# cokwa/bitHTM

Hardware: AMD Instinct MI355X
Metric: HTM timesteps/sec (SP + TM, learning on), 65536 cols x 32 cells (higher is better)
Workload: dtype u32 bit-packed / f64 + f32 permanences; 1 GPU; configs[2]: 65536 columns x 32 cells, SP + TM learning on, 1 MI355X; input_dim=1024, column_dim=65536, cell_dim=32, active_columns=1311, patterns=50, pretrain_steps=500, segments=96476, segment_slots=128, hip_graph=True, hip_graph_requested=True, pipelined=True, repetitions=15, streamed_calls=True

## Files before the change

bithtm_amd/_lib.py:

```python

import ctypes as C
import os

HERE = os.path.dirname(os.path.abspath(__file__))
LIB_PATH = os.path.join(HERE, "libbithtm_hip.so")
ABI_VERSION = 4


class HtmConfig(C.Structure):
    _fields_ = [
        ("struct_bytes", C.c_uint32), ("device", C.c_int32),
        ("input_dim", C.c_int32), ("column_dim", C.c_int32), ("cell_dim", C.c_int32),
        ("active_columns", C.c_int32), ("enable_sp", C.c_int32), ("enable_tm", C.c_int32),
        ("sp_permanence_threshold", C.c_double), ("sp_delta_on", C.c_double), ("sp_delta_off", C.c_double),
        ("boost_coefficient", C.c_float), ("duty_momentum", C.c_float), ("duty_increment", C.c_float),
        ("tm_learn_active", C.c_double), ("tm_learn_inactive", C.c_double),
        ("tm_punish_active", C.c_double), ("tm_punish_inactive", C.c_double),
        ("tm_learn_prune", C.c_int32), ("tm_punish_prune", C.c_int32),
        ("tm_permanence_initial", C.c_float), ("tm_permanence_threshold", C.c_float),
        ("segment_activation_threshold", C.c_int32), ("segment_matching_threshold", C.c_int32),
        ("segment_sampling_synapses", C.c_int32),
        ("segment_capacity", C.c_int32), ("segment_capacity_local", C.c_int32), ("segment_slots", C.c_int32),
        ("seed", C.c_uint32), ("shard_rank", C.c_int32), ("shard_world", C.c_int32), ("use_caller_stream", C.c_int32),
        ("stream", C.c_void_p),
    ]


class HtmInfo(C.Structure):
    _fields_ = [
        ("step_index", C.c_int64), ("segments", C.c_int32), ("local_segments", C.c_int32), ("matching_segments", C.c_int32),
        ("winner_cells", C.c_int32), ("active_cells", C.c_int32), ("has_distal_state", C.c_int32),
        ("has_winner_cells", C.c_int32), ("capacity_error", C.c_int32), ("words_per_row", C.c_int32),
        ("new_segment_requests", C.c_int32), ("recycled_segments", C.c_int32), ("appended_segments", C.c_int32),
        ("work_items", C.c_int32), ("select_fallbacks", C.c_int32), ("candidate_exact_steps", C.c_int32), ("hot_select_steps", C.c_int32),
        ("select_zoom_steps", C.c_int32),
    ]


class HtmStepRecord(C.Structure):
    _fields_ = [(name, C.c_int32) for name in (
        "active_columns", "bursting_columns", "predicted_columns_before", "predicted_columns", "active_cells", "winner_cells",
        "segments", "new_segments")]


class HtmRunRecord(C.Structure):
    _fields_ = [("struct_bytes", C.c_uint32), ("records", C.c_void_p), ("active_column", C.c_void_p), ("column_prediction", C.c_void_p)]


F_ACTIVE_COLUMN, F_OVERLAPS, F_BOOSTED, F_DUTY_CYCLE, F_CELL_ACTIVATION, F_CELL_PREDICTION = 1, 2, 3, 4, 5, 6
F_WINNER_WORDS, F_BURSTING, F_WINNER_CELL, F_SEG_CELL, F_SEG_NSYN, F_SEG_PRESYN, F_SEG_PERM = 7, 8, 9, 10, 11, 12, 13
F_SEGCOUNT, F_SEG_POTENTIAL, F_MATCH_SEGMENT, F_MATCH_INFO, F_MATCH_JITTER, F_CELL_MAX_JITTER = 14, 15, 16, 17, 18, 19
F_SEG_GID = 20
PLAN_GRAPH, PLAN_PIPELINED, PLAN_LEAN, PLAN_SCAN_LARGE = 1, 2, 4, 8
SP_OVERLAP, SP_BOOST, SP_SELECT, SP_ACTIVE, SP_LEARN, SP_DUTY, SP_COMMIT = 1, 2, 3, 4, 5, 6, 7

EXPORTS = {
    "htm_abi_version": (C.c_int, []),
    "htm_create": (C.c_int, [C.POINTER(HtmConfig), C.POINTER(C.c_void_p)]),
    "htm_destroy": (None, [C.c_void_p]),
    "htm_last_error": (C.c_char_p, [C.c_void_p]),
    "htm_sp_set_permanence": (C.c_int, [C.c_void_p, C.c_void_p, C.c_int32, C.c_int32]),
    "htm_set_epsilon": (C.c_int, [C.c_void_p, C.c_float]),
    "htm_sp_get_permanence": (C.c_int, [C.c_void_p, C.c_void_p, C.c_int32, C.c_int32]),
    "htm_step": (C.c_int, [C.c_void_p, C.c_void_p, C.c_int32]),
    "htm_sp_step": (C.c_int, [C.c_void_p, C.c_void_p, C.c_int32]),
    "htm_sp_phase": (C.c_int, [C.c_void_p, C.c_int32, C.c_void_p, C.c_int64]),
    "htm_tm_step": (C.c_int, [C.c_void_p, C.c_void_p, C.c_int32, C.c_int32, C.c_int32]),
    "htm_tm_update": (C.c_int, [C.c_void_p, C.c_void_p, C.c_void_p, C.c_void_p, C.c_int32, C.c_void_p]),
    "htm_tm_scan": (C.c_int, [C.c_void_p, C.c_void_p]),
    "htm_tm_run": (C.c_int, [C.c_void_p, C.c_void_p, C.c_int32, C.c_int32, C.c_int32, C.c_int32, C.c_int32, C.POINTER(HtmRunRecord)]),
    "htm_run": (C.c_int, [C.c_void_p, C.c_void_p, C.c_int32, C.c_int32, C.c_int32, C.c_int32]),
    "htm_prepare": (C.c_int, [C.c_void_p, C.c_void_p, C.c_int32, C.c_int32, C.c_int32, C.c_int32]),
    "htm_run_recorded": (C.c_int, [C.c_void_p, C.c_void_p, C.c_int32, C.c_int32, C.c_int32, C.c_int32, C.POINTER(HtmRunRecord)]),
    "htm_prepare_recorded": (C.c_int, [C.c_void_p, C.c_void_p, C.c_int32, C.c_int32, C.c_int32, C.c_int32]),
    "htm_reset": (C.c_int, [C.c_void_p]),
    "htm_set_run_resets": (C.c_int, [C.c_void_p, C.c_void_p, C.c_int32]),
    "htm_predicted_input": (C.c_int, [C.c_void_p, C.c_void_p]),
    "htm_set_run_predicted_input": (C.c_int, [C.c_void_p, C.c_void_p]),
    "htm_graph_count": (C.c_int, [C.c_void_p]),
    "htm_run_plan": (C.c_int, [C.c_void_p, C.c_int32, C.c_int32]),
    "htm_bank_upload": (C.c_int, [C.c_void_p, C.c_void_p, C.c_int32, C.POINTER(C.c_void_p)]),
    "htm_shard_record_bytes": (C.c_int64, [C.c_void_p]),
    "htm_shard_begin": (C.c_int, [C.c_void_p, C.c_void_p, C.c_int32, C.c_void_p, C.c_int32, C.c_void_p]),
    "htm_shard_finish": (C.c_int, [C.c_void_p, C.c_void_p, C.c_int32]),
    "htm_shard_unique_id": (C.c_int, [C.c_void_p]),
    "htm_shard_comm_init": (C.c_int, [C.c_void_p, C.c_void_p]),
    "htm_shard_step": (C.c_int, [C.c_void_p, C.c_void_p, C.c_int32, C.c_void_p, C.c_int32]),
    "htm_shard_comm_size": (C.c_int, [C.c_void_p]),
    "htm_shard_graph_ok": (C.c_int, [C.c_void_p]),
    "htm_shard_run": (C.c_int, [C.c_void_p, C.c_void_p, C.c_int32, C.c_int32, C.c_int32, C.c_int32]),
    "htm_shard_group_run": (C.c_int, [C.POINTER(C.c_void_p), C.c_int32, C.POINTER(C.c_void_p), C.c_int32, C.c_int32, C.c_int32, C.c_int32]),
    "htm_rccl_selftest": (C.c_int, [C.c_int32]),
    "htm_keyed_draws": (C.c_int, [C.c_uint32, C.c_int32, C.c_uint32, C.c_void_p, C.c_void_p, C.c_int64, C.c_void_p]),
    "htm_shard_group_step": (C.c_int, [C.POINTER(C.c_void_p), C.c_int32, C.POINTER(C.c_void_p), C.c_int32, C.c_void_p, C.c_int32]),
    "htm_populate": (C.c_int, [C.c_void_p, C.c_int64, C.c_int64, C.c_int32, C.c_int32, C.c_double, C.c_double, C.c_uint32]),
    "htm_sync": (C.c_int, [C.c_void_p]),
    "htm_get_stream": (C.c_int, [C.c_void_p, C.POINTER(C.c_void_p)]),
    "htm_get_info": (C.c_int, [C.c_void_p, C.POINTER(HtmInfo)]),
    "htm_read": (C.c_int64, [C.c_void_p, C.c_int32, C.c_void_p, C.c_int64]),
    "htm_read_rows": (C.c_int64, [C.c_void_p, C.c_int32, C.c_int64, C.c_int64, C.c_void_p, C.c_int64]),
    "htm_import_begin": (C.c_int, [C.c_void_p, C.c_int64]),
    "htm_write": (C.c_int, [C.c_void_p, C.c_int32, C.c_void_p, C.c_int64]),
    "htm_import_commit": (C.c_int, [C.c_void_p, C.c_int32, C.c_int32, C.c_int32, C.c_int32, C.c_int32]),
    "htm_profile": (C.c_int, [C.c_void_p, C.c_int32]),
    "htm_profile_read": (C.c_int, [C.c_void_p, C.c_int32, C.POINTER(C.c_char_p), C.POINTER(C.c_double),
                                   C.POINTER(C.c_int64)]),
    "htm_trace_read": (C.c_int64, [C.c_void_p, C.c_void_p, C.c_int64]),
    "htm_group_create": (C.c_int, [C.POINTER(C.c_void_p), C.c_int32, C.POINTER(C.c_void_p)]),
    "htm_group_destroy": (None, [C.c_void_p]),
    "htm_group_last_error": (C.c_char_p, [C.c_void_p]),
    "htm_group_run": (C.c_int, [C.c_void_p, C.POINTER(C.c_void_p), C.c_int32, C.c_int32, C.c_int32, C.c_int32, C.POINTER(HtmRunRecord)]),
    "htm_group_step": (C.c_int, [C.c_void_p, C.c_void_p, C.c_int32, C.POINTER(HtmRunRecord)]),
    "htm_create_view": (C.c_int, [C.c_void_p, C.POINTER(C.c_void_p)]),
    "htm_device_bytes": (C.c_int64, [C.c_void_p]),
    "htm_pack_columns": (C.c_int, [C.c_void_p, C.c_void_p, C.c_int32, C.c_int32, C.c_int32, C.c_void_p, C.c_int32, C.c_int32]),
    "htm_encode_votes": (C.c_int, [C.c_void_p, C.c_int32, C.c_int32, C.c_void_p, C.c_int32, C.c_int32]),
    "htm_set_run_feedback": (C.c_int, [C.c_void_p, C.c_void_p, C.c_int32, C.c_int32, C.c_int32]),
}

HIP_EXPORTS = {
    "hipSetDevice": (C.c_int, [C.c_int]),
    "hipMalloc": (C.c_int, [C.POINTER(C.c_void_p), C.c_size_t]),
    "hipFree": (C.c_int, [C.c_void_p]),
    "hipMemcpy": (C.c_int, [C.c_void_p, C.c_void_p, C.c_size_t, C.c_int]),
    "hipGetErrorString": (C.c_char_p, [C.c_int]),
    "hipStreamCreateWithFlags": (C.c_int, [C.POINTER(C.c_void_p), C.c_uint]),
    "hipStreamDestroy": (C.c_int, [C.c_void_p]),
}
HIP_MEMCPY_HOST_TO_DEVICE = 1
HIP_MEMCPY_DEVICE_TO_HOST = 2

_lib = None


def load():
# ... 21 lines not shown
```

bithtm_amd/csrc/htm_dev.h:

```cpp
#ifndef BITHTM_HTM_DEV_H
#define BITHTM_HTM_DEV_H

typedef unsigned long long u64;

#define SEL_MAX_PASSES 6
#define SEL_DIGIT 12
#define SEL_BINS 4096
#define HIST_REP 4
#define SEL_COARSE 64
#define COARSE_REP 16
#define COARSE_STRIDE 1024
#define FAN_COUNTERS 16
#define FAN_STRIDE 32
#define HIST0_FINE (HIST_REP * SEL_BINS)
#define HIST0_PAR (HIST0_FINE + COARSE_REP * COARSE_STRIDE)
#define RB 512
#define SCAN_SEGS 64
#define DEAD_CAP 256
#define SHARD_HOT_KEYS 4
#define CAND_CAP 256
#define WIN_LDS 4096
#define MAX_SLOTS 512
#define SYN_CONNECTED 0x80000000u
#define SYN_CELL 0x7FFFFFFF
#define SEG_BUSY 0x40000000
#define EPS32 1e-8f

#define KEY_SHIFT 3
__device__ __forceinline__ u64 select_key_bits(u64 bits) { return bits ? (bits - ((u64)(1023 - 150) << 52)) << KEY_SHIFT : 0ull; }
__device__ __forceinline__ u64 select_key(double boosted) { return select_key_bits((u64)__double_as_longlong(boosted)); }

#define WIN_COARSE 31
#define WIN_FINE 7
#define WIN_BINS (2 + (WIN_COARSE << WIN_FINE))
#define WIN_LOWBITS (52 - WIN_FINE)
static_assert(WIN_BINS <= SEL_BINS, "the window's bins fit the select histogram");
__host__ __device__ __forceinline__ uint32_t win_bin(u64 key, uint32_t base) {
    const uint32_t c = (uint32_t)(key >> 52);
    if (c < base) return 0u;
    const uint32_t o = c - base;
    return o >= WIN_COARSE ? 1u + (WIN_COARSE << WIN_FINE) : 1u + ((o << WIN_FINE) | ((uint32_t)(key >> WIN_LOWBITS) & ((1u << WIN_FINE) - 1u)));
}
__host__ __device__ __forceinline__ uint32_t win_base_for(u64 kth_key) {
    const uint32_t c = (uint32_t)(kth_key >> 52);
    return c > WIN_COARSE / 2 ? min(c - WIN_COARSE / 2, 4096u - WIN_COARSE) : 0u;
}

__host__ __device__ __forceinline__ uint32_t win_base_global(u64 kth_key) { return win_base_for(kth_key); }

__host__ __device__ __forceinline__ int sel_shift(int pass) { return pass < 5 ? 52 - SEL_DIGIT * pass : 0; }
__host__ __device__ __forceinline__ int sel_bits(int pass) { return pass < 5 ? SEL_DIGIT : 4; }

struct Counters {
    uint32_t step[2];
    int32_t S;
    int32_t n_win[2];
    int32_t has_winner[2];
    int32_t has_distal;
    uint32_t cm_dense_step;
    int32_t n_active_cells;
    alignas(128) int32_t n_work[2];
    int32_t n_bind[2];
    alignas(128) int32_t n_work_last;
    int32_t sel_fallbacks;
    int32_t cand_exact;
    int32_t hot_selects;
    int32_t sel_zooms;
    uint32_t emit_epoch;
    int32_t n_un;
    int32_t n_recycled, n_new, S_old;
    int32_t L;
    int32_t n_lfree;
    int32_t error;
    u64 sel_prefix[2];
    uint32_t sel_krem[2];
    uint32_t sel_win[2];
    uint32_t sel_win_global;
    u64 sel_pass_prefix[2][SEL_MAX_PASSES + 1];
    uint32_t sel_pass_krem[2][SEL_MAX_PASSES + 1];
};

struct Dev {
    int I, W, W4, Ipad, C, K, k, E, Scap, work_cap, sel_passes, colwords, low_zero, cand_d, cand_pairwise, cand_others, cand_speculate, cand_take_all, cand_zoom, poll_delay;
    int win_offset;
    int cls_rows_max;
    int LK, KP, WPC;
    int world, c0, c1;
    int sel_lo, sel_hi, sel_k;
    int Lcap, n_cand;
    int hot_budget, hot_target;
    int cand_cap;
    double sp_thr, sp_don, sp_doff;
    float coef, mom, dinc;
    double lrn_act, lrn_inact, pun_act, pun_inact;
    int lrn_prune, pun_prune;
    float perm_init, perm_thr;
    float eps;
    int act_thr, match_thr, sample;
    uint32_t seed;
    double *perm;
    uint32_t *mask;
    float *duty;
    int *overlap[2];
    double *boosted[2];
    u64 *key[2];
    uint32_t *hist;
    uint32_t *hist0;
    uint32_t *sel_blk;
    uint32_t *sel_rec;
    int *active_cols[2];
    uint32_t *input_stage;
    uint32_t *act[2];
    uint32_t *pred[2];
    uint32_t *win[2];
    uint32_t *colbits[2];
    int *winners[2];
    uint8_t *bursting;
    int *actw_id;
    uint32_t *winw_idx;
    uint8_t *actcnt;
    uint32_t *act_list;
    uint16_t *col_rank[2];
    uint32_t *unacc_word;
    uint32_t *fan;
    int *unacc_list;
    int *seg_cell;
    int *seg_nsyn;
    int *presyn;
    float *sperm;
    int *segcount;
    uint32_t *cellmax[2];
    uint32_t *match_bits[2];
    uint32_t *seg_info;
    float *seg_jit;
    uint32_t *work;
    int *recyc_cnt;
    int *recyc_cnt2;
    int *recyc_need;
    int *seg_gid;
    int *g2l;
    uint32_t *dead_bits;
    int *lfree;
    int *asg_gid;
    int *cand_cols;
    int *dead_list;
    const uint32_t *punish;
    unsigned char *send;
    Counters *ctr;
    unsigned long long *trace;
    uint32_t trace_until;
};

__device__ __forceinline__ int lane_id() { return threadIdx.x & 63; }
__device__ __forceinline__ u64 lanemask_lt() { return (1ull << lane_id()) - 1ull; }

__device__ __forceinline__ uint32_t wave_incl_scan(uint32_t v) {
    uint32_t t = v;
    t += (uint32_t)__builtin_amdgcn_update_dpp(0, (int)v, 0x111, 0xf, 0xf, false);
    t += (uint32_t)__builtin_amdgcn_update_dpp(0, (int)v, 0x112, 0xf, 0xf, false);
    t += (uint32_t)__builtin_amdgcn_update_dpp(0, (int)v, 0x113, 0xf, 0xf, false);
    t += (uint32_t)__builtin_amdgcn_update_dpp(0, (int)t, 0x114, 0xf, 0xe, false);
    t += (uint32_t)__builtin_amdgcn_update_dpp(0, (int)t, 0x118, 0xf, 0xc, false);
    t += (uint32_t)__builtin_amdgcn_update_dpp(0, (int)t, 0x142, 0xa, 0xf, false);
    t += (uint32_t)__builtin_amdgcn_update_dpp(0, (int)t, 0x143, 0xc, 0xf, false);
    return t;
}

__device__ __forceinline__ uint32_t wave_sum(uint32_t v) { return (uint32_t)__builtin_amdgcn_readlane((int)wave_incl_scan(v), 63); }

#ifdef BITHTM_BISECT_A
__device__ __forceinline__ uint32_t wave_read(uint32_t v, int src) { return (uint32_t)__shfl((int)v, src); }
__device__ __forceinline__ int wave_read(int v, int src) { return __shfl(v, src); }
#else
__device__ __forceinline__ uint32_t wave_read(uint32_t v, int src) { return (uint32_t)__builtin_amdgcn_readlane((int)v, src); }
__device__ __forceinline__ int wave_read(int v, int src) { return __builtin_amdgcn_readlane(v, src); }
#endif
__device__ __forceinline__ u64 wave_read(u64 v, int src) {
#ifdef BITHTM_BISECT_A
    return ((u64)(uint32_t)__shfl((int)(v >> 32), src) << 32) | (uint32_t)__shfl((int)(uint32_t)v, src);
#endif
    return ((u64)(uint32_t)__builtin_amdgcn_readlane((int)(v >> 32), src) << 32) | (uint32_t)__builtin_amdgcn_readlane((int)(uint32_t)v, src);
}

template <typename Op>
// ... 36 lines not shown
__device__ __forceinline__ void lds_barrier() { asm volatile("s_waitcnt lgkmcnt(0)\n\ts_barrier" ::: "memory"); }

template <typename Op>
__device__ __forceinline__ float half_reduce(float v, float ident, Op op) {
    const int id = __float_as_int(ident);
#define BITHTM_DPPF(src, ctrl, rm, bm) __int_as_float(__builtin_amdgcn_update_dpp(id, __float_as_int(src), ctrl, rm, bm, false))
    float t = v;
    t = op(t, BITHTM_DPPF(v, 0x111, 0xf, 0xf));
    t = op(t, BITHTM_DPPF(v, 0x112, 0xf, 0xf));
    t = op(t, BITHTM_DPPF(v, 0x113, 0xf, 0xf));
    t = op(t, BITHTM_DPPF(t, 0x114, 0xf, 0xe));
    t = op(t, BITHTM_DPPF(t, 0x118, 0xf, 0xc));
    t = op(t, BITHTM_DPPF(t, 0x142, 0xa, 0xf));
#undef BITHTM_DPPF
    const float lo = __int_as_float(__builtin_amdgcn_readlane(__float_as_int(t), 31));
    const float hi = __int_as_float(__builtin_amdgcn_readlane(__float_as_int(t), 63));
    return lane_id() < 32 ? lo : hi;
}

template <int BS, bool LDS_ONLY = false>
__device__ __forceinline__ uint32_t block_excl_scan(uint32_t v, uint32_t *s_wave, uint32_t &total) {
    const int lane = lane_id(), wv = threadIdx.x >> 6;
    const uint32_t x = wave_incl_scan(v);
    if (lane == 63) s_wave[wv] = x;
    if (LDS_ONLY) lds_barrier(); else __syncthreads();
    uint32_t woff = 0, tot = 0;
#pragma unroll
    for (int i = 0; i < BS / 64; ++i) {
        uint32_t t = s_wave[i];
        if (i < wv) woff += t;
        tot += t;
    }
    if (LDS_ONLY) lds_barrier(); else __syncthreads();
    total = tot;
    return woff + x - v;
}

__device__ __forceinline__ int wave_append(int *counter, bool pred) {
    u64 m = __ballot(pred);
    if (m == 0) return -1;
    int leader = __ffsll((long long)m) - 1;
    int base = 0;
    if (lane_id() == leader) base = atomicAdd(counter, __popcll(m));
    base = wave_read(base, leader);
    return pred ? base + __popcll(m & lanemask_lt()) : -1;
}

__device__ __forceinline__ void recyc_add(const Dev &d, int blk1024, int delta) {
    atomicAdd(&d.recyc_cnt[blk1024], delta);
    atomicAdd(&d.recyc_cnt2[blk1024 >> 10], delta);
}

__device__ __forceinline__ void hist_add(uint32_t *h, uint32_t digit, bool active) {
    u64 todo = __ballot(active);
    while (todo) {
        const int leader = __ffsll((long long)todo) - 1;
        const uint32_t dl = wave_read(digit, leader);
        const u64 same = __ballot(active && digit == dl) & todo;
        if (lane_id() == leader) atomicAdd(&h[dl], (uint32_t)__popcll(same));
        todo &= ~same;
    }
}

__device__ __forceinline__ void hist_add_tie(uint32_t *h, uint32_t digit, bool active) {
    const u64 act = __ballot(active);
    if (!act) return;
    const int leader = __ffsll((long long)act) - 1;
    const uint32_t dl = wave_read(digit, leader);
    const u64 same = __ballot(active && digit == dl);
    if (lane_id() == leader) atomicAdd(&h[dl], (uint32_t)__popcll(same));
    if (active && digit != dl) atomicAdd(&h[digit], 1u);
}

__device__ __forceinline__ u64 spread32(uint32_t v) {
    u64 x = v;
    x = (x | (x << 16)) & 0x0000FFFF0000FFFFull;
    x = (x | (x << 8)) & 0x00FF00FF00FF00FFull;
    x = (x | (x << 4)) & 0x0F0F0F0F0F0F0F0Full;
    x = (x | (x << 2)) & 0x3333333333333333ull;
    x = (x | (x << 1)) & 0x5555555555555555ull;
    return x;
}

__device__ __forceinline__ uint32_t cell_mask(int K) { return K >= 32 ? 0xFFFFFFFFu : ((1u << K) - 1u); }
__device__ __forceinline__ u64 cell_mask64(int K) { return K >= 64 ? ~0ull : ((1ull << K) - 1ull); }
__device__ __forceinline__ uint32_t cell_mask_word(int K, int h) { return cell_mask(K - 32 * h); }
__device__ __forceinline__ uint32_t enc_to_flat(const Dev &d, int enc) { return (uint32_t)((enc >> d.LK) * d.K + (enc & (d.KP - 1))); }

#endif
```

bithtm_amd/csrc/htm_engine.hip:

```cpp

#include <hip/hip_runtime.h>
#include <hip/hip_ext.h>
#include <dlfcn.h>
#include <stdint.h>
#include <stdio.h>
#include <string.h>
#include <algorithm>
#include <climits>
#include <chrono>
#include <map>
#include <mutex>
#include <string>
#include <tuple>
#include <type_traits>
#include <vector>

#include "../../include/bithtm_hip.h"
#include "htm_fexp.h"
#include "htm_rng.h"

#include "htm_dev.h"
#include "htm_sp_kernels.h"
#include "htm_tm_kernels.h"
#include "htm_pipeline.h"
#include "htm_record.h"
#include "htm_reset.h"
#include "htm_decode.h"
#include "htm_stack.h"
#include "htm_forecast.h"
#include "htm_group.h"
#include "htm_tm_feed.h"


struct ncclUniqueIdBytes { char internal[128]; };

static thread_local std::string g_create_error;
static int (*g_rccl_destroy)(void *) = nullptr;

struct Knobs {
    int graph_steps, eager_below;
    bool trace;
    uint32_t trace_until;
    int lean, lean2_classify, lean2_order, step_split, fuse_tm, shard_window, step_window, tail_rows, scan_large, scan_large_above, scan_dyn;
    int defer_tail, shared_scan, shared_members;
    int lean_overlap, lean_learn, lean_learn_large, lean_scan, lean_scan_large, scan_blocks, sel_launch_digits;
    int cand_d, cand_pairwise, cls_rows_max, win_offset, cand_zoom, cand_speculate, cand_take_all, poll_delay, cand_others;
};

struct Sizes {
    int G;
    int sp_blocks, sel_blocks, c256_blocks, s1024_blocks, scan_blocks, zero_blocks, cus;
    int lean_learn_blocks, lean_learn_blocks_large, lean_scan_blocks, lean_scan_blocks_large, lean_overlap_blocks, lean2_classify_blocks;
    int lean_resident_large;
    bool emit_fits, emit_fits_open;
    bool emit_fits_lean;
    int sel_passes_fused, sel_passes_full;
};

struct RunGraphKey {
    int p; bool recording, resetting, decoding, feeding; int learning; bool sp_done, next_sp, next_front, lean; int spec; bool large, emit_fused, wmode;
    int span; const void *bank; int n_inputs;
    auto tie() const { return std::tie(p, recording, resetting, decoding, feeding, learning, sp_done, next_sp, next_front, lean, spec, large, emit_fused, wmode, span, bank, n_inputs); }
    bool operator<(const RunGraphKey &o) const { return tie() < o.tie(); }
};

struct ShardGraphKey {
    int p, learning; bool front_done, front_next; int span, ranks, n_inputs; std::vector<std::tuple<int, bool, bool>> per_rank; const void *bank;
    auto tie() const { return std::tie(p, learning, front_done, front_next, span, ranks, n_inputs, per_rank, bank); }
    bool operator<(const ShardGraphKey &o) const { return tie() < o.tie(); }
};

struct TmRunGraphKey {
    int p; bool recording, resetting; int learning, spec; bool large; int span; const void *lists; int n_rows, n;
    auto tie() const { return std::tie(p, recording, resetting, learning, spec, large, span, lists, n_rows, n); }
    bool operator<(const TmRunGraphKey &o) const { return tie() < o.tie(); }
};

struct htm_handle {
    htm_config cfg;
    Dev d;
    Knobs knob;
    Sizes sz;
    int device;
    hipStream_t stream;
    bool own_stream;
    long long step_host;
    std::string err;
    std::vector<void *> allocs;
    int *d_cols_stage;
    int rank, world;
    const uint32_t *shard_bank;
    int shard_n_inputs = 1;
    bool shard_open;
    bool shard_graph_ok;
    int shard_front_wmode;
    std::map<ShardGraphKey, hipGraphExec_t> shard_graphs;
    void *rccl_comm;
    unsigned char *shard_send, *shard_recv;
    bool emit_fused, emit_fused_open;
    bool tail_pending;
    int tail_p;
    bool window_known;
    int seg_hint;
    int *seg_pinned;
    const uint32_t *ahead_bank;
    int ahead_n_inputs, ahead_learning;
    bool ahead_lean;
    int phase_active;
    bool import_keep;
    bool phase_open;
    RecDev *d_rec;
    bool recording;
    const uint32_t *reset_bits;
    int reset_n;
    ResetDev *d_reset;
    bool resetting;
    int32_t *pin_out;
    PinDev *d_pin;
    bool decoding;
    int32_t *d_pin_buf;
    uint32_t *feed_bank;
    int feed_n;
    FeedDev *d_feed;
    int32_t *d_feed_votes;
    bool feeding;
    std::map<RunGraphKey, hipGraphExec_t> graphs;
    std::map<TmRunGraphKey, hipGraphExec_t> tm_graphs;
    std::vector<int> imp_pot, imp_match_seg;
    std::vector<int> imp_seg_cell, imp_seg_nsyn, imp_presyn;
    std::vector<float> imp_perm;
    std::vector<uint32_t> imp_match_info;
    std::vector<float> imp_match_jit;
    bool profile;
    hipEvent_t prof_last;
    std::vector<hipEvent_t> prof_all;
// ... 217 lines not shown
        LAUNCH_ON(h, h->stream, lds, "tm_learn+tm_scan", kt_lse_plain[epl_slot(d)], n_learn + n_scan, 256, d, p, 0, n_learn, n_scan, spec);
    } else {
        launch_learn(h, p);
        launch_scan(h, p, scan_lds(d, 1) <= 64 * 1024);
    }
}

static void flush_tail(htm_handle *h) {
    if (!h->tail_pending) return;
    h->tail_pending = false;
    hipSetDevice(h->device);
    enqueue_tm_tail(h, h->tail_p);
}

static decltype(&k_learn_scan_tail<1>) const kt_learn_scan_tail[4] = {k_learn_scan_tail<1>, k_learn_scan_tail<2>, k_learn_scan_tail<4>, k_learn_scan_tail<8>};

static void enqueue_tm(htm_handle *h, int n_active, int learning, int want_winner, int p,
                       const uint32_t *bank, int n_inputs, bool sp_rows, int front_wmode = -1, bool defer_tail = false) {
    Dev &d = h->d;
    const int n_cls = learning ? kClassifyBlocks : 0;
    const bool fuse = tm_tail_fused(h);
    int n_sp_rows = (sp_rows && learning && h->cfg.enable_sp) ? d.k : 0;
    const int n_tail_rows = (fuse && h->world == 1 && h->knob.tail_rows && !defer_tail) ? n_sp_rows : 0;
    if (n_tail_rows) n_sp_rows = 0;
    const int n_duty = h->world > 1 ? (d.c1 - d.c0 + 255) / 256 : 0;
    LAUNCH(h, "tm_mid", k_mid_rows, 1 + n_cls + n_sp_rows + n_duty + h->sz.zero_blocks, 256, d, p, n_active, want_winner, learning, n_cls, bank, n_inputs, n_sp_rows, 0, n_duty);
    if (defer_tail) { h->tail_pending = true; h->tail_p = p; return; }
    if (fuse && (front_wmode >= 0 || n_tail_rows)) {
        const int epl = learn_epl(d), n_learn = h->sz.lean_learn_blocks, n_scan = h->sz.lean_scan_blocks, spec = scan_spec_blocks(h);
        const size_t lds = std::max(std::max(learn_lds(epl, 256), scan_lds(d, 1)), (size_t)SEL_BINS * 4);
        const int grid = n_learn + n_scan + (n_tail_rows ? n_tail_rows : h->sz.lean_overlap_blocks);
        const char *name = n_tail_rows ? "tm_learn+tm_scan+sp_learn" : "tm_learn+tm_scan+shard_overlap";
        LAUNCH_ON(h, h->stream, lds, name, kt_learn_scan_tail[epl_slot(d)], grid, 256, d, p, n_learn, n_scan, spec, bank, n_inputs, h->sz.G, front_wmode, n_tail_rows);
        return;
    }
    enqueue_tm_tail(h, p);
    if (front_wmode >= 0)
        LAUNCH(h, "shard_overlap", k_shard_overlap, h->sz.sp_blocks, RB, d, bank, n_inputs, h->sz.G, p, front_wmode, 1);
}

struct StepPlan { bool sp_done, next_sp, next_front; };

static bool can_pipeline(const htm_handle *h) {
    return h->cfg.enable_sp && h->cfg.enable_tm && h->world == 1 && h->emit_fused_open && h->d.sel_passes == 2;
}

static bool can_lean(const htm_handle *h) {
    return h->knob.lean && can_pipeline(h) && scan_lds(h->d, 1) <= 64 * 1024 && h->sz.emit_fits_lean;
}

static decltype(&k_learn_scan_emit<1, 6>) const kt_lse_large[4] = {k_learn_scan_emit<1, 4, false>, k_learn_scan_emit<2, 4, false>,
                                                                   k_learn_scan_emit<4, 4, false>, k_learn_scan_emit<8, 4, false>};
static decltype(&k_learn_scan_emit<1, 6>) const kt_lse_tab[4] = {k_learn_scan_emit<1, 6, true>, k_learn_scan_emit<2, 6, true>,
                                                                 k_learn_scan_emit<4, 6, true>, k_learn_scan_emit<8, 6, true>};
static decltype(&k_learn_scan_emit<1, 6>) lse_kernel(const Dev &d, int form) {
    return (form == LSE_TAB ? kt_lse_tab : form == LSE_LARGE ? kt_lse_large : kt_lse_plain)[epl_slot(d)];
}

static int lse_form(const htm_handle *h) { return scan_pool_is_large(h) ? LSE_LARGE : lean_tab(h->d) ? LSE_TAB : LSE_PLAIN; }

static void launch_learn_scan_emit(htm_handle *h, int p, int n_emit) {
    Dev &d = h->d;
    const int epl = learn_epl(d);
    const size_t lds = std::max(std::max(learn_lds(epl, 256), lean_scan_lds(d)), sizeof(EmitShared));
    const bool large = scan_pool_is_large(h), dyn = large && h->knob.scan_dyn > 0;
    const int n_learn = dyn ? h->sz.lean_learn_blocks_large : h->sz.lean_learn_blocks;
    int n_scan = large ? h->sz.lean_scan_blocks_large : h->sz.lean_scan_blocks;
    if (dyn) n_scan = std::max(64, h->sz.lean_resident_large - n_emit - n_learn);
    const int grid = n_emit + n_learn + n_scan;
    if (large && !dyn) n_scan = -n_scan;
    const int spec = dyn ? 0 : scan_spec_blocks(h);
    const char *lse_name = large ? "tm_learn+tm_scan_large+sp_emit" : "tm_learn+tm_scan+sp_emit";
    LAUNCH_ON(h, h->stream, lds, lse_name, lse_kernel(d, lse_form(h)), grid, 256, d, p, n_emit, n_learn, n_scan, spec);
}

static int lean2_classify_blocks(const htm_handle *h, int learning) {
    if (!learning) return 0;
    return scan_pool_is_large(h) && !h->knob.lean2_classify ? std::max(h->sz.lean2_classify_blocks, 192) : h->sz.lean2_classify_blocks;
}

static void enqueue_lean(htm_handle *h, int p, int learning, const uint32_t *bank, int n_inputs, StepPlan plan) {
    Dev &d = h->d;
    const int n_act = (d.k * d.KP + 255) / 256, n_rows = learning ? d.k : 0;
    const int n_cls = learning ? kClassifyBlocks : 0, n_ov = plan.next_sp ? h->sz.lean_overlap_blocks : 0;
    if (h->knob.lean == 2) {
        const int n_cls2 = lean2_classify_blocks(h, learning);
        const int n_duty = n_ov ? 0 : h->sz.c256_blocks, n_clear = d.WPC * h->sz.c256_blocks;
        LAUNCH_ON(h, h->stream, (size_t)SEL_BINS * 4, "tm_activate+tm_mid+sp_learn+sp_overlap", k_act_mid_rows,
                  n_act + 1 + n_cls2 + n_rows + n_ov + n_duty + n_clear + h->sz.zero_blocks, 256, d, p, d.k, n_act, learning, n_cls2, bank, n_inputs, n_rows, h->sz.G, n_ov,
                  n_duty, n_clear, h->knob.lean2_order);
    } else {
        LAUNCH(h, "tm_activate+sp_learn", k_act_rows, n_act + n_rows + (1 + d.WPC) * h->sz.c256_blocks, 256, d, p, d.k, n_act, bank, n_inputs, n_rows, h->sz.c256_blocks);
        LAUNCH_ON(h, h->stream, (size_t)SEL_BINS * 4, "tm_mid+sp_overlap", k_mid_overlap, 1 + n_cls + n_ov + h->sz.zero_blocks, 256, d, p, d.k, 1, learning, n_cls,
                  bank, n_inputs, h->sz.G, n_ov);
    }
    launch_learn_scan_emit(h, p, plan.next_sp ? h->sz.c256_blocks : 0);
}

static decltype(&k_learn_overlap<1>) const kt_learn_overlap[4] = {k_learn_overlap<1>, k_learn_overlap<2>, k_learn_overlap<4>, k_learn_overlap<8>};
static decltype(&k_scan_sel<true, 1>) const kt_scan_sel[4] = {k_scan_sel<true, 1>, k_scan_sel<false, 1>, k_scan_sel<true, 6>, k_scan_sel<false, 6>};

static void enqueue_pipelined(htm_handle *h, int p, int learning, const uint32_t *bank, int n_inputs, StepPlan plan) {
    Dev &d = h->d;
    const int n_cls = learning ? kClassifyBlocks : 0;
    const int n_emit = plan.next_sp ? h->sz.c256_blocks : 0;
    LAUNCH_ON(h, h->stream, sizeof(EmitShared), "tm_activate+sp_emit", k_open_emit, n_emit + (d.k * d.KP + 255) / 256, 256, d, p, n_emit, d.k);
    const int n_rows = (plan.next_sp && learning) ? d.k : 0, n_duty = plan.next_sp ? h->sz.c256_blocks : 0;
    LAUNCH(h, "tm_mid+sp_learn", k_mid_rows, 1 + n_cls + n_rows + n_duty + h->sz.zero_blocks, 256, d, p, d.k, 1, learning, n_cls, bank, n_inputs, n_rows, 1, n_duty);
    LAUNCH_ON(h, h->stream, std::max(learn_lds(learn_epl(d)), (size_t)SEL_BINS * 4), "tm_learn+sp_overlap", kt_learn_overlap[epl_slot(d)],
              kLearnBlocks + (plan.next_front ? h->sz.sp_blocks : 0), RB, d, p, kLearnBlocks, bank, n_inputs, h->sz.G, p, 2);
    const bool use_lds = scan_lds(d, 1) <= 64 * 1024, large = scan_pool_is_large(h);
    const int n_sel = plan.next_front ? 64 : 0, n_clear = plan.next_sp ? h->sz.c256_blocks : 0;
    LAUNCH_ON(h, h->stream, std::max(scan_lds(d, use_lds), sizeof(SelShared)), large ? "tm_scan_large+sp_select" : "tm_scan+sp_select",
              kt_scan_sel[scan_slot(large, use_lds)], h->sz.scan_blocks + n_sel + n_clear, 256, d, p, n_sel, n_clear, p, scan_spec_blocks(h));
}

static void enqueue_cold_start(htm_handle *h, const uint32_t *bank, int n_inputs, int learning, StepPlan plan) {
    Dev &d = h->d;
    const int p = (int)(h->step_host & 1);
    if (plan.sp_done || !plan.next_sp) return;
    const int wmode = step_wmode(h);
    if (can_lean(h)) {
        enqueue_sp_front(h, bank, n_inputs, p, wmode);
        enqueue_sp_back(h, bank, n_inputs, p, 1, 0, false, wmode);
        return;
    }
    enqueue_sp_front(h, bank, n_inputs, p, wmode);
    enqueue_sp_back(h, bank, n_inputs, p, 1, EMIT_DUTY | EMIT_CLEAR, learning != 0, wmode);
    LAUNCH(h, "sp_overlap", k_sp_overlap, h->sz.sp_blocks, RB, d, bank, n_inputs, h->sz.G, p, p ^ 1, 1, 0);
    LAUNCH(h, "sp_select", k_sel_pass, h->sz.sel_blocks, RB, d, 1, p ^ 1);
}

static int reset_blocks(const Dev &d) { return std::max(1, std::min(1024, (d.C * d.KP + 255) / 256)); }

static void enqueue_run_reset(htm_handle *h, int p) {
    if (h->resetting) LAUNCH(h, "tm_reset", k_tm_reset, reset_blocks(h->d), 256, h->d, p, h->d_reset, h->recording ? h->d_rec : nullptr, 0u);
}

static void enqueue_rest(htm_handle *h, int p, const uint32_t *bank, int n_inputs, int learning, StepPlan plan) {
    enqueue_run_reset(h, p);
    if ((plan.sp_done || plan.next_sp) && can_lean(h)) {
        enqueue_lean(h, p, learning, bank, n_inputs, plan);
    } else if (plan.sp_done || plan.next_sp) {
        enqueue_pipelined(h, p, learning, bank, n_inputs, plan);
    } else {
        enqueue_sp_back(h, bank, n_inputs, p, 1, EMIT_ALL, false, step_wmode(h));
        enqueue_tm(h, h->d.k, learning, 1, p, bank, n_inputs, true);
    }
}

static int rec_blocks(const Dev &d) { return std::max(REC_BLOCKS_MIN, (d.k + 255) / 256); }

static void enqueue_record(htm_handle *h, int p) {
    if (h->recording) LAUNCH(h, "record", k_rec_step, rec_blocks(h->d), 256, h->d, p, h->d_rec);
}

static void enqueue_decode(htm_handle *h, int p) {
    if (h->decoding) LAUNCH(h, "predicted_input", k_pin_step, pin_blocks(h->d.C), 256, h->d, p, (const PinDev *)h->d_pin);
}

static bool decode_unpipelined(const htm_handle *h) { return h->pin_out && !can_lean(h); }

static void enqueue_feed(htm_handle *h, int p) {
    if (!h->feeding) return;
    LAUNCH(h, "feedback_votes", k_feed_votes, pin_blocks(h->d.C), 256, h->d, p, (const FeedDev *)h->d_feed);
    LAUNCH(h, "feedback_encode", k_feed_step, 1, ENC_THREADS, h->d, p, (const FeedDev *)h->d_feed);
}

static int pin_begin_blocks(int n, int I) { return (int)std::max<size_t>(1, std::min<size_t>(1024, ((size_t)n * I + 255) / 256)); }

static int enqueue_step(htm_handle *h, const uint32_t *bank, int n_inputs, int learning, StepPlan plan, const uint32_t *host_input = nullptr) {
    if (!plan.sp_done && !plan.next_sp) enqueue_sp_front(h, bank, n_inputs, (int)(h->step_host & 1), step_wmode(h), host_input);
    enqueue_cold_start(h, bank, n_inputs, learning, plan);
    enqueue_rest(h, (int)(h->step_host & 1), bank, n_inputs, learning, plan);
    enqueue_record(h, (int)(h->step_host & 1));
    enqueue_decode(h, (int)(h->step_host & 1));
    enqueue_feed(h, (int)(h->step_host & 1));
    h->step_host += 1;
    return launch_status(h->err);
}

extern "C" int htm_abi_version(void) { return BITHTM_ABI_VERSION; }

extern "C" const char *htm_last_error(const htm_handle *h) { return h ? h->err.c_str() : g_create_error.c_str(); }

extern "C" void htm_destroy(htm_handle *h) {
    if (!h) return;
    {
        std::lock_guard<std::mutex> lock(g_registry_mutex);
        g_registry.erase(std::remove(g_registry.begin(), g_registry.end(), h), g_registry.end());
    }
    hipSetDevice(h->device);
    hipStreamSynchronize(h->stream);
    for (auto &kv : h->graphs) hipGraphExecDestroy(kv.second);
    for (auto &kv : h->shard_graphs) hipGraphExecDestroy(kv.second);
    for (auto &kv : h->tm_graphs) hipGraphExecDestroy(kv.second);
    for (auto &v : h->prof_events)
        for (auto &pr : v) { hipEventDestroy(pr.first); hipEventDestroy(pr.second); }
    for (hipEvent_t e : h->prof_all) hipEventDestroy(e);
    if (h->rccl_comm && g_rccl_destroy) g_rccl_destroy(h->rccl_comm);
    for (void *p : h->allocs) hipFree(p);
    for (void *p : h->weight_allocs) hipFree(p);
    if (h->seg_pinned) hipHostFree(h->seg_pinned);
    if (h->own_stream) hipStreamDestroy(h->stream);
    if (HtmShared *sh = h->shared) {
        bool last;
        {
            std::lock_guard<std::mutex> lock(g_shared_mutex);
            if (sh->parent == h) sh->parent = nullptr;
            last = --sh->refs == 0;
        }
        if (last) {
            for (void *p : sh->allocs) hipFree(p);
            if (sh->own_stream) hipStreamDestroy(sh->stream);
            delete sh;
        }
    }
    delete h;
}

static int fail_create(htm_handle *h, const std::string &msg, int code) {
    g_create_error = msg;
    if (h) { h->err = msg; htm_destroy(h); }
    return code;
}

static int alloc_weights(htm_handle *h) {
    Dev &d = h->d;
    const htm_config *cfg = &h->cfg;
    const size_t C = d.C;
    int rc = 0;
    if (cfg->enable_sp) {
        rc |= dalloc_weights(h, &d.perm, C * d.Ipad);
        rc |= dalloc_weights(h, &d.mask, C * d.W);
    }
    if (cfg->enable_tm) {
        const size_t S = d.Lcap, E = d.E, KP = d.KP;
        rc |= dalloc_weights(h, &d.seg_cell, S);
        rc |= dalloc_weights(h, &d.seg_nsyn, S);
        rc |= dalloc_weights(h, &d.presyn, S * E);
        rc |= dalloc_weights(h, &d.sperm, S * E);
        rc |= dalloc_weights(h, &d.segcount, C * KP);
    }
    return rc;
}

static int alloc_stream_state(htm_handle *h) {
    Dev &d = h->d;
    const htm_config *cfg = &h->cfg;
    const int world = h->world;
    int rc = 0;
    const size_t C = d.C, k = d.k;
    rc |= dalloc(h, &d.ctr, 1);
    rc |= dalloc(h, &d.active_cols[0], k + 8);
    rc |= dalloc(h, &d.active_cols[1], k + 8);
    if (cfg->enable_sp) {
        rc |= dalloc(h, &d.duty, C);
        for (int q = 0; q < 2; ++q) {
            rc |= dalloc(h, &d.overlap[q], C);
            rc |= dalloc(h, &d.boosted[q], C);
            rc |= dalloc(h, &d.key[q], C);
        }
        rc |= dalloc(h, &d.hist, (size_t)2 * SEL_MAX_PASSES * SEL_BINS);
        rc |= dalloc(h, &d.hist0, (size_t)2 * HIST0_PAR);
        rc |= dalloc(h, &d.sel_blk, (C + 255) / 256);
        rc |= dalloc(h, &d.sel_rec, (C + 255) / 256 * 32);
        rc |= dalloc(h, &d.input_stage, (size_t)d.W);
    }
    if (cfg->enable_tm) {
        const size_t S = d.Lcap, G = d.Scap;
        const size_t KP = d.KP, WPC = d.WPC;
        for (int q = 0; q < 2; ++q) {
            rc |= dalloc(h, &d.act[q], C * WPC);
            rc |= dalloc(h, &d.pred[q], C * WPC);
            rc |= dalloc(h, &d.winners[q], k * KP);
        }
        rc |= dalloc(h, &d.win[0], C * WPC);
        rc |= dalloc(h, &d.win[1], C * WPC);
        d.colwords = (int)((C + 63) / 64) * 2;
        const size_t colwords_padded = (size_t)((C + 255) / 256) * 8;
        rc |= dalloc(h, &d.colbits[0], colwords_padded);
        rc |= dalloc(h, &d.colbits[1], colwords_padded);
        rc |= dalloc(h, &d.bursting, k);
        rc |= dalloc(h, &d.actw_id, k * WPC + 8);
        rc |= dalloc(h, &d.winw_idx, k * WPC + 8);
        rc |= dalloc(h, &d.actcnt, k * WPC + 8);
        rc |= dalloc(h, &d.act_list, k * WPC + 16);
        rc |= dalloc(h, &d.col_rank[0], colwords_padded);
        rc |= dalloc(h, &d.col_rank[1], colwords_padded);
        rc |= dalloc(h, &d.unacc_word, k * WPC + 8);
        rc |= dalloc(h, &d.fan, (size_t)2 * FAN_COUNTERS * FAN_STRIDE);
        rc |= dalloc(h, &d.unacc_list, k * KP);
        for (int q = 0; q < 2; ++q) {
            rc |= dalloc(h, &d.cellmax[q], C * KP);
            rc |= dalloc(h, &d.match_bits[q], (S + 255) / 256 * 8);
        }
        rc |= dalloc(h, &d.seg_info, S);
        rc |= dalloc(h, &d.seg_jit, S);
        rc |= dalloc(h, &d.work, (size_t)d.work_cap);
        rc |= dalloc(h, &d.recyc_cnt, (G + 1023) / 1024);
        rc |= dalloc(h, &d.recyc_cnt2, ((G + 1023) / 1024 + 1023) / 1024 + 1);
        rc |= dalloc(h, &d.recyc_need, 2 * k * KP);
        rc |= dalloc(h, &d.dead_list, (size_t)1 + DEAD_CAP);
        if (world > 1) {
            rc |= dalloc(h, &d.seg_gid, S);
            rc |= dalloc(h, &d.g2l, G);
            rc |= dalloc(h, &d.dead_bits, (G + 31) / 32 + 32);
            rc |= dalloc(h, &d.lfree, S);
            rc |= dalloc(h, &d.asg_gid, k * 32);
            rc |= dalloc(h, &d.cand_cols, (size_t)d.n_cand + 8);
            if (!rc && (hipMemsetAsync(d.seg_gid, 0xFF, S * 4, h->stream) != hipSuccess ||
                        hipMemsetAsync(d.g2l, 0xFF, G * 4, h->stream) != hipSuccess)) { h->err = "hipMemsetAsync failed"; rc = HTM_ERR_HIP; }
        }
        rc |= dalloc(h, &h->d_cols_stage, k);
    }
    if (h->knob.trace) rc |= dalloc(h, &d.trace, (size_t)8 * 4096 * 2);
    return rc;
}

static const char *env_str(const char *name) { return getenv(name); }
static int env_int(const char *name, int dflt, int lo = INT_MIN, int hi = INT_MAX) {
    const char *e = env_str(name);
    return e ? std::max(lo, std::min(hi, atoi(e))) : dflt;
}
static int env_flag(const char *name, int dflt) {
    const char *e = env_str(name);
    return e ? atoi(e) != 0 : dflt;
}

static Knobs read_knobs() {
    Knobs k;
    k.graph_steps = env_int("BITHTM_GRAPH_STEPS", 16, 1, 256);
    k.eager_below = env_int("BITHTM_EAGER_BELOW", 64, 0);
    k.trace = env_str("BITHTM_TRACE") != nullptr;
    const char *until = env_str("BITHTM_TRACE_UNTIL");
    k.trace_until = until ? (uint32_t)strtoul(until, nullptr, 10) : 0xFFFFFFFFu;
    k.lean = env_int("BITHTM_LEAN", 2, 0, 2);
    k.lean2_classify = env_int("BITHTM_LEAN2_CLASSIFY", 0, 1);
    k.step_split = env_flag("BITHTM_STEP_SPLIT", 1);
    {
        const char *e = env_str("BITHTM_LEAN2_ORDER");
        const int o = e ? (int)strtol(e, nullptr, 16) : 0x0312;
        int seen = 0, pos[4] = {-1, -1, -1, -1};
        for (int i = 0; i < 4; ++i) { const int r = (o >> (4 * (3 - i))) & 15; if (r < 4) { seen |= 1 << r; pos[r] = i; } }
        k.lean2_order = (o >= 0 && o <= 0x3333 && seen == 15 && pos[0] < pos[1]) ? o : 0x0312;
    }
    k.fuse_tm = env_flag("BITHTM_FUSE_TM", 1);
    k.shard_window = env_flag("BITHTM_SHARD_WINDOW", 1);
    k.scan_large = env_int("BITHTM_SCAN_LARGE", -1);
    k.scan_large_above = env_int("BITHTM_SCAN_LARGE_ABOVE", 3 * 1536 * SCAN_SEGS, 0);
    k.step_window = env_flag("BITHTM_STEP_WINDOW", 1);
    k.tail_rows = env_flag("BITHTM_TAIL_ROWS", 1);
    k.scan_dyn = env_flag("BITHTM_SCAN_DYN", 1);
    k.defer_tail = env_flag("BITHTM_DEFER_TAIL", 1);
    k.shared_scan = env_flag("BITHTM_SHARED_SCAN", 0);
    k.shared_members = env_int("BITHTM_SHARED_SCAN_MEMBERS", 0, 0);
    k.lean_overlap = env_int("BITHTM_LEAN_OVERLAP", 0, 1);
    k.lean_learn = env_int("BITHTM_LEAN_LEARN", 0, 1);
    k.lean_learn_large = env_int("BITHTM_LEAN_LEARN_LARGE", 0, 1);
    k.lean_scan = env_int("BITHTM_LEAN_SCAN", 0, 1);
    k.lean_scan_large = env_int("BITHTM_LEAN_SCAN_LARGE", 0, 1);
    k.scan_blocks = env_int("BITHTM_SCAN_BLOCKS", 0, 1);
    k.sel_launch_digits = env_int("BITHTM_SEL_LAUNCH_DIGITS", -1, 0);
    k.cand_d = env_int("BITHTM_CAND_D", CAND_D, 0, CAND_D);
    k.cand_pairwise = env_int("BITHTM_CAND_PAIRWISE", CAND_PAIRWISE, 0);
    k.cls_rows_max = env_int("BITHTM_CLASSIFY_WORDS_ABOVE", -1, 0);
    k.win_offset = env_int("BITHTM_SEL_WINDOW_OFFSET", 0, 0);
    k.cand_zoom = env_int("BITHTM_CAND_ZOOM", -1);
    k.cand_speculate = env_flag("BITHTM_CAND_SPECULATE", 1);
    k.cand_take_all = env_flag("BITHTM_CAND_TAKE_ALL", 1);
    k.poll_delay = env_int("BITHTM_POLL_DELAY", 7, 0, 64);
    k.cand_others = env_int("BITHTM_CAND_OTHERS", CAND_OTHERS, 0, CAND_OTHERS);
    return k;
}

static void size_launches(htm_handle *h) {
    Dev &d = h->d;
    const Knobs &k = h->knob;
    Sizes &z = h->sz;
    z.G = 1;
    while (z.G < d.W4 && z.G < 64) z.G <<= 1;
    const int rows_per_block = (RB / 64) * 4 * (64 / z.G);
    z.sp_blocks = std::max(1, std::min((d.c1 - d.c0 + rows_per_block - 1) / rows_per_block, 256));
    z.sel_blocks = std::max(1, std::min((d.sel_hi - d.sel_lo + RB - 1) / RB, 128));
    z.c256_blocks = (d.sel_hi - d.sel_lo + 255) / 256;
    z.s1024_blocks = std::max(1, (d.Scap + 1023) / 1024);
    z.scan_blocks = std::max(1, std::min((d.Lcap + SCAN_SEGS - 1) / SCAN_SEGS, 2048));
    if (z.scan_blocks > 256) z.scan_blocks = (z.scan_blocks + 255) & ~255;
    z.zero_blocks = std::max(1, std::min((d.Lcap / 128 + 4095) / 4096, 1024));
    z.lean_overlap_blocks = k.lean_overlap ? k.lean_overlap : z.sp_blocks * (RB / 256);
    z.lean_learn_blocks = k.lean_learn ? k.lean_learn : 512;
    z.lean_learn_blocks_large = k.lean_learn_large ? k.lean_learn_large : k.lean_learn ? z.lean_learn_blocks : 768;
    z.lean_scan_blocks = k.lean_scan ? k.lean_scan : (z.scan_blocks > 512 ? std::max(256, (z.scan_blocks * 3 / 8 + 255) & ~255) : z.scan_blocks);
    z.lean_scan_blocks_large = k.lean_scan_large ? k.lean_scan_large : k.lean_scan ? z.lean_scan_blocks : z.scan_blocks;
    if (k.scan_blocks) z.scan_blocks = k.scan_blocks;
    hipDeviceProp_t prop;
    const bool have_prop = hipGetDeviceProperties(&prop, h->device) == hipSuccess;
    z.cus = have_prop ? prop.multiProcessorCount : 256;
    int B = 0;
    while ((1ll << B) <= (long long)d.I) ++B;
    const int informative = std::min(64, 64 - (29 - B) - KEY_SHIFT);
    d.sel_passes = std::max(1, std::min(SEL_MAX_PASSES, (informative + SEL_DIGIT - 1) / SEL_DIGIT));
    d.low_zero = 64 - informative;
    int per_cu_emit = 0, per_cu_open = 0;
    if (have_prop && hipOccupancyMaxActiveBlocksPerMultiprocessor(&per_cu_emit, (const void *)k_sp_emit, 256, 0) == hipSuccess &&
        hipOccupancyMaxActiveBlocksPerMultiprocessor(&per_cu_open, (const void *)k_open_emit, 256, sizeof(EmitShared)) == hipSuccess) {
        z.emit_fits = z.c256_blocks <= std::min(1024, per_cu_emit * z.cus);
        z.emit_fits_open = z.emit_fits && z.c256_blocks + (d.k * d.KP + 255) / 256 <= std::min(1024, per_cu_open * z.cus);
        int per_cu_lean = 1 << 30;
        z.lean_resident_large = 1 << 30;
        const size_t lean_lds = std::max(std::max(learn_lds(learn_epl(d), 256), lean_scan_lds(d)), sizeof(EmitShared));
        bool asked = h->cfg.enable_tm && z.emit_fits && lean_lds <= 64 * 1024;
        for (int form = LSE_TAB; asked && form <= LSE_LARGE; ++form) {
            if (form == LSE_TAB && !lean_tab(d)) continue;
            int per_cu = 0;
            asked = hipOccupancyMaxActiveBlocksPerMultiprocessor(&per_cu, (const void *)lse_kernel(d, form), 256, lean_lds) == hipSuccess;
            per_cu_lean = std::min(per_cu_lean, per_cu);
            if (asked && form == LSE_LARGE) z.lean_resident_large = per_cu * z.cus;
        }
        z.emit_fits_lean = asked && z.c256_blocks <= std::min(1024, per_cu_lean * z.cus);
        if (z.lean_resident_large == (1 << 30)) z.lean_resident_large = 4 * z.cus;
    } else {
        (void)hipGetLastError();
        z.emit_fits = z.emit_fits_open = z.emit_fits_lean = false;
        z.lean_resident_large = 1024;
    }
    if (k.lean2_classify) {
        z.lean2_classify_blocks = k.lean2_classify;
    } else {
        int per_cu = 0, resident = 1536;
        if (have_prop && hipOccupancyMaxActiveBlocksPerMultiprocessor(&per_cu, (const void *)k_act_mid_rows, 256, (size_t)SEL_BINS * 4) == hipSuccess)
            resident = per_cu * z.cus;
        else
            (void)hipGetLastError();
        const int others = (d.k * d.KP + 255) / 256 + z.lean_overlap_blocks + d.k + 1;
        const int room = (resident - others) & ~7;
        z.lean2_classify_blocks = room >= 128 ? std::min(kClassifyBlocks, room) : 32;
    }
    z.sel_passes_full = d.sel_passes;
    z.sel_passes_fused = std::min(d.sel_passes, 2);
    if (k.sel_launch_digits >= 0) z.sel_passes_fused = std::max(2, std::min(d.sel_passes, k.sel_launch_digits));
}

extern "C" int htm_create(const htm_config *cfg, htm_handle **out) {
    if (!cfg || !out) return fail_create(nullptr, "htm_create: null argument", HTM_ERR_ARGUMENT);
    if (cfg->struct_bytes != sizeof(htm_config)) return fail_create(nullptr, "htm_create: htm_config size mismatch (ABI)", HTM_ERR_ARGUMENT);
    if (cfg->column_dim < 1 || cfg->active_columns < 1 || cfg->active_columns > cfg->column_dim)
        return fail_create(nullptr, "htm_create: need 1 <= active_columns <= column_dim", HTM_ERR_ARGUMENT);
    if (cfg->enable_sp && cfg->input_dim < 1) return fail_create(nullptr, "htm_create: input_dim < 1", HTM_ERR_ARGUMENT);
    if (cfg->enable_tm) {
        if (cfg->cell_dim < 1 || cfg->cell_dim > 64) return fail_create(nullptr, "htm_create: cell_dim must be in 1..64", HTM_ERR_ARGUMENT);
        if (cfg->segment_slots < 64 || cfg->segment_slots > MAX_SLOTS || cfg->segment_slots % 64)
            return fail_create(nullptr, "htm_create: segment_slots must be a multiple of 64 in 64..512", HTM_ERR_ARGUMENT);
        if (cfg->segment_capacity < 1) return fail_create(nullptr, "htm_create: segment_capacity < 1", HTM_ERR_ARGUMENT);
        if (cfg->segment_sampling_synapses < 1 || cfg->segment_sampling_synapses > 64)
            return fail_create(nullptr, "htm_create: segment_sampling_synapses must be in 1..64", HTM_ERR_ARGUMENT);
        if (cfg->segment_activation_threshold < cfg->segment_matching_threshold)
            return fail_create(nullptr, "htm_create: activation threshold < matching threshold", HTM_ERR_ARGUMENT);
        if ((long long)cfg->column_dim * (cfg->cell_dim > 32 ? 64 : 32) > 0x7FFFFFFFLL) return fail_create(nullptr, "htm_create: column_dim too large", HTM_ERR_ARGUMENT);
    }
    if (!cfg->enable_sp && !cfg->enable_tm) return fail_create(nullptr, "htm_create: nothing enabled", HTM_ERR_ARGUMENT);
    const int world = cfg->shard_world > 1 ? cfg->shard_world : 1;
    if (world > 1) {
        if (!cfg->enable_sp || !cfg->enable_tm) return fail_create(nullptr, "htm_create: a sharded handle needs SP and TM", HTM_ERR_ARGUMENT);
        if (cfg->cell_dim > 32) return fail_create(nullptr, "htm_create: a sharded handle takes cell_dim up to 32 (the exchange record carries one 32-bit word per column)", HTM_ERR_ARGUMENT);
        if (world > 64) return fail_create(nullptr, "htm_create: at most 64 shards", HTM_ERR_ARGUMENT);
        if (cfg->shard_rank < 0 || cfg->shard_rank >= world) return fail_create(nullptr, "htm_create: shard_rank out of range", HTM_ERR_ARGUMENT);
        if (cfg->column_dim % (world * 64)) return fail_create(nullptr, "htm_create: column_dim must be a multiple of 64 * shard_world", HTM_ERR_ARGUMENT);
    }

    htm_handle *h = new htm_handle();
    h->cfg = *cfg;
    h->device = cfg->device;
    h->rank = world > 1 ? cfg->shard_rank : 0;
    h->world = world;
    h->knob = read_knobs();
    hipError_t e = hipSetDevice(cfg->device);
    if (e != hipSuccess) return fail_create(h, std::string("hipSetDevice: ") + hipGetErrorString(e), HTM_ERR_HIP);
    if (cfg->use_caller_stream) {
        h->stream = (hipStream_t)cfg->stream;
    } else {
        e = hipStreamCreateWithFlags(&h->stream, hipStreamNonBlocking);
        if (e != hipSuccess) return fail_create(h, std::string("hipStreamCreate: ") + hipGetErrorString(e), HTM_ERR_HIP);
        h->own_stream = true;
    }
    Dev &d = h->d;
    d.I = cfg->enable_sp ? cfg->input_dim : 0;
    d.W = ((d.I + 127) / 128) * 4;
    d.W4 = d.W / 4;
    d.Ipad = d.W * 32;
    d.C = cfg->column_dim;
    d.world = world;
    d.c0 = h->rank * (d.C / world);
    d.c1 = d.c0 + d.C / world;
    d.K = cfg->enable_tm ? cfg->cell_dim : 0;
    d.KP = d.K > 32 ? 64 : 32;
    d.LK = d.K > 32 ? 6 : 5;
    d.WPC = d.KP / 32;
    d.k = cfg->active_columns;
    d.E = cfg->enable_tm ? cfg->segment_slots : 64;
    d.Scap = cfg->enable_tm ? cfg->segment_capacity : 0;
    d.Lcap = d.Scap;
    if (world > 1) {
        const long long dflt = std::min<long long>(d.Scap, 2LL * d.Scap / world + 1024);
        d.Lcap = cfg->segment_capacity_local > 0 ? std::min(cfg->segment_capacity_local, cfg->segment_capacity) : (int)dflt;
    }
    d.work_cap = d.Lcap + d.k * d.KP;
    d.sel_lo = d.c0; d.sel_hi = d.c1;
    d.sel_k = d.n_cand = std::min(d.k, d.c1 - d.c0);
    d.cand_cap = shard_cand_cap(d.n_cand, d.c1 - d.c0);
    d.hot_budget = std::max(1, std::min(d.cand_cap, (SHARD_HOT_KEYS * 1024) / std::max(world, 1)));
    d.hot_target = std::max(1, std::min(d.sel_k, d.hot_budget / 2));
    d.sp_thr = cfg->sp_permanence_threshold; d.sp_don = cfg->sp_delta_on; d.sp_doff = cfg->sp_delta_off;
    d.coef = cfg->boost_coefficient; d.mom = cfg->duty_momentum; d.dinc = cfg->duty_increment;
    d.lrn_act = cfg->tm_learn_active; d.lrn_inact = cfg->tm_learn_inactive;
    d.pun_act = cfg->tm_punish_active; d.pun_inact = cfg->tm_punish_inactive;
    d.lrn_prune = cfg->tm_learn_prune; d.pun_prune = cfg->tm_punish_prune;
    d.perm_init = cfg->tm_permanence_initial; d.perm_thr = cfg->tm_permanence_threshold;
    d.eps = EPS32;
    d.act_thr = cfg->segment_activation_threshold; d.match_thr = cfg->segment_matching_threshold;
    d.sample = cfg->segment_sampling_synapses;
    d.seed = cfg->seed;
    const Knobs &k = h->knob;
    d.trace_until = k.trace_until; d.cand_d = k.cand_d; d.cand_pairwise = k.cand_pairwise; d.cls_rows_max = k.cls_rows_max; d.win_offset = k.win_offset;
    d.cand_zoom = k.cand_zoom; d.cand_speculate = k.cand_speculate; d.cand_take_all = k.cand_take_all; d.poll_delay = k.poll_delay; d.cand_others = k.cand_others;
    int rc = alloc_weights(h);
    rc |= alloc_stream_state(h);
    if (rc) return fail_create(h, h->err, HTM_ERR_HIP);
    if (hipHostMalloc((void **)&h->seg_pinned, sizeof(int), hipHostMallocDefault) == hipSuccess) *h->seg_pinned = 0; else h->seg_pinned = nullptr;
    size_launches(h);
    e = hipStreamSynchronize(h->stream);
    if (e != hipSuccess) return fail_create(h, std::string("hipStreamSynchronize: ") + hipGetErrorString(e), HTM_ERR_HIP);
    {
        std::lock_guard<std::mutex> lock(g_registry_mutex);
        g_registry.push_back(h);
    }
    refresh_exchange_mode(h);
    *out = h;
    return HTM_OK;
}


#define REFUSE_ON_VIEW(h, what)                                                                                   \
    do {                                                                                                          \
        if ((h)->is_view) {                                                                                       \
            (h)->err = std::string(what) + ": not available on an inference view (it shares its parent's weights and never learns)"; \
            return HTM_ERR_STATE;                                                                                 \
        }                                                                                                         \
    } while (0)

static void weights_touched(htm_handle *h) {
    if (h->shared && !h->is_view) {
        std::lock_guard<std::mutex> lock(g_shared_mutex);
        h->shared->wgen += 1;
    }
}

static int view_enter(htm_handle *h, int learning) {
    if (!h->is_view) return 0;
    if (learning) { h->err = "an inference view steps with learning = 0 only (it shares its parent's weights)"; return HTM_ERR_STATE; }
    htm_handle *par;
    long long wgen;
    {
        std::lock_guard<std::mutex> lock(g_shared_mutex);
        par = h->shared->parent;
        wgen = h->shared->wgen;
    }
    HIPCHK(h, hipSetDevice(h->device));
    if (par) {
        flush_tail(par);
        if (sp_is_ahead(par)) {
            h->err = "the view's parent is ahead (its htm_run ended with HTM_RUN_CONTINUE): finish the parent's run first";
            return HTM_ERR_STATE;
        }
// ... 73 lines not shown
              hipMemsetAsync(d.ctr->n_bind, 0, sizeof(d.ctr->n_bind), h->stream) == hipSuccess &&
              hipMemsetAsync(&d.ctr->error, 0, sizeof(int32_t), h->stream) == hipSuccess;
    if (ok) {
        hipLaunchKernelGGL(k_tm_reset, dim3(reset_blocks(d)), dim3(256), 0, h->stream, d, (int)(h->step_host & 1), (const ResetDev *)nullptr,
                           (RecDev *)nullptr, (uint32_t)h->step_host);
        ok = hipGetLastError() == hipSuccess;
    }
    if (hipHostMalloc((void **)&h->seg_pinned, sizeof(int), hipHostMallocDefault) == hipSuccess) *h->seg_pinned = parent->seg_hint; else h->seg_pinned = nullptr;
    if (!ok || hipStreamSynchronize(h->stream) != hipSuccess) return fail_create(h, "htm_create_view: copying the parent's stream state failed", HTM_ERR_HIP);
    {
        std::lock_guard<std::mutex> lock(g_registry_mutex);
        g_registry.push_back(h);
    }
    refresh_exchange_mode(h);
    *out = h;
    return HTM_OK;
}

extern "C" int64_t htm_device_bytes(htm_handle *h) {
    if (!h) return HTM_ERR_ARGUMENT;
    return h->own_bytes;
}

extern "C" int htm_set_epsilon(htm_handle *h, float epsilon) {
    if (!h) return HTM_ERR_ARGUMENT;
    if (h) flush_tail(h);
    if (!(epsilon > 0.f) || epsilon > 1.f) { h->err = "htm_set_epsilon: need 0 < epsilon <= 1"; return HTM_ERR_ARGUMENT; }
    REJECT_WHEN_AHEAD(h);
    if (epsilon == h->d.eps) return HTM_OK;
    HIPCHK(h, hipSetDevice(h->device));
    HIPCHK(h, hipStreamSynchronize(h->stream));
    for (auto &kv : h->graphs) hipGraphExecDestroy(kv.second);
    h->graphs.clear();
    h->d.eps = epsilon;
    return HTM_OK;
}

extern "C" int htm_get_stream(htm_handle *h, void **stream) {
    if (!h || !stream) return HTM_ERR_ARGUMENT;
    *stream = (void *)h->stream;
    return HTM_OK;
}

extern "C" int htm_sync(htm_handle *h) {
    if (!h) return HTM_ERR_ARGUMENT;
    if (h) flush_tail(h);
    HIPCHK(h, hipSetDevice(h->device));
    const auto t0 = std::chrono::steady_clock::now();
    for (;;) {
        const hipError_t e = hipStreamQuery(h->stream);
        if (e == hipSuccess) return HTM_OK;
        if (e != hipErrorNotReady) { h->err = std::string("hipStreamQuery: ") + hipGetErrorString(e); return HTM_ERR_HIP; }
        if (std::chrono::steady_clock::now() - t0 > std::chrono::milliseconds(2)) break;
    }
    HIPCHK(h, hipStreamSynchronize(h->stream));
    return HTM_OK;
}

static int check_rows(htm_handle *h, const void *rows, int row_begin, int row_count) {
    if (!h) return HTM_ERR_ARGUMENT;
    if (!h->cfg.enable_sp) { h->err = "handle has no Spatial Pooler"; return HTM_ERR_STATE; }
    if (!rows || row_begin < 0 || row_count < 0 || row_begin + (long long)row_count > h->d.C) {
        h->err = "permanence rows out of range";
        return HTM_ERR_ARGUMENT;
    }
    return 0;
}

extern "C" int htm_sp_set_permanence(htm_handle *h, const double *rows, int32_t row_begin, int32_t row_count) {
    if (h) REFUSE_ON_VIEW(h, "htm_sp_set_permanence");
    if (h) flush_tail(h);
    if (h) weights_touched(h);
    int rc = check_rows(h, rows, row_begin, row_count);
    if (rc) return rc;
    REJECT_WHEN_AHEAD(h);
    if (row_count == 0) return HTM_OK;
    Dev &d = h->d;
    HIPCHK(h, hipSetDevice(h->device));
    HIPCHK(h, hipMemcpy2DAsync(d.perm + (size_t)row_begin * d.Ipad, (size_t)d.Ipad * 8, rows, (size_t)d.I * 8,
                               (size_t)d.I * 8, (size_t)row_count, hipMemcpyHostToDevice, h->stream));
    const long long waves = (long long)row_count * (d.Ipad / 64);
    const int blocks = (int)std::min<long long>((waves + 3) / 4, 8192);
    hipLaunchKernelGGL(k_sp_build_mask, dim3(blocks), dim3(256), 0, h->stream, d, row_begin, row_count);
    HIPCHK(h, hipStreamSynchronize(h->stream));
    return HTM_OK;
}

extern "C" int htm_sp_get_permanence(htm_handle *h, double *rows, int32_t row_begin, int32_t row_count) {
    if (h) flush_tail(h);
    int rc = check_rows(h, rows, row_begin, row_count);
    if (rc) return rc;
    REJECT_WHEN_AHEAD(h);
    if (row_count == 0) return HTM_OK;
    Dev &d = h->d;
    HIPCHK(h, hipSetDevice(h->device));
    HIPCHK(h, hipMemcpy2DAsync(rows, (size_t)d.I * 8, d.perm + (size_t)row_begin * d.Ipad, (size_t)d.Ipad * 8,
                               (size_t)d.I * 8, (size_t)row_count, hipMemcpyDeviceToHost, h->stream));
    HIPCHK(h, hipStreamSynchronize(h->stream));
    return HTM_OK;
}

static int close_open_phases(htm_handle *h) {
    if (!h->phase_open) return 0;
    const int p = (int)(h->step_host & 1);
    if (h->cfg.enable_sp) HIPCHK(h, hipMemsetAsync(h->d.hist0 + (size_t)p * HIST0_PAR, 0, (size_t)HIST0_PAR * 4, h->stream));
    h->phase_open = false;
    h->phase_active = 0;
    return 0;
}

static int stage_input(htm_handle *h, const uint32_t *packed_input) {
    Dev &d = h->d;
    const int words = (d.I + 31) / 32;
    HIPCHK(h, hipMemcpyAsync(d.input_stage, packed_input, (size_t)words * 4, hipMemcpyHostToDevice, h->stream));
    return 0;
}

static decltype(&k_learn_scan_front<1>) const kt_learn_scan_front[4] = {k_learn_scan_front<1>, k_learn_scan_front<2>, k_learn_scan_front<4>, k_learn_scan_front<8>};

extern "C" int htm_step(htm_handle *h, const uint32_t *packed_input, int32_t learning) {
    if (!h || !packed_input) return HTM_ERR_ARGUMENT;
    REJECT_WHEN_AHEAD(h);
    if (!h->cfg.enable_sp || !h->cfg.enable_tm) { h->err = "htm_step needs a handle with SP and TM"; return HTM_ERR_STATE; }
    if (h->world > 1) { h->err = "sharded handle: use htm_shard_begin / htm_shard_finish"; return HTM_ERR_STATE; }
    HIPCHK(h, hipSetDevice(h->device));
    int rc = view_enter(h, learning);
    if (rc) return rc;
    if (learning) weights_touched(h);
    refresh_exchange_mode(h);
    rc = close_open_phases(h);
    if (rc) return rc;
    if (h->d.W > ARG_INPUT_WORDS) {
        flush_tail(h);
        rc = stage_input(h, packed_input);
        if (rc) return rc;
    }
    Dev &d = h->d;
    if (h->knob.defer_tail && d.W <= ARG_INPUT_WORDS && tm_tail_fused(h) && !h->profile) {
        const int p = (int)(h->step_host & 1), wmode = step_wmode(h);
        const bool ride_emit = h->knob.step_split && h->tail_pending && wmode && h->emit_fused && can_lean(h);
        bool emitted = false;
        if (ride_emit) {
            enqueue_sp_front(h, d.input_stage, 1, p, wmode, packed_input);
            h->tail_pending = false;
            launch_learn_scan_emit(h, h->tail_p, h->sz.c256_blocks);
            h->window_known = true;
            emitted = true;
        } else if (h->tail_pending) {
            PackedInputArg in;
            memset(&in, 0, sizeof(in));
            memcpy(in.w, packed_input, (size_t)((d.I + 31) / 32) * 4);
            const int epl = learn_epl(d), n_learn = h->sz.lean_learn_blocks, n_scan = h->sz.lean_scan_blocks, spec = scan_spec_blocks(h);
            const size_t lds = std::max(std::max(learn_lds(epl, 256), scan_lds(d, 1)), (size_t)(SEL_BINS + ARG_INPUT_WORDS) * 4);
            const int grid = n_learn + n_scan + h->sz.lean_overlap_blocks;
            h->tail_pending = false;
            LAUNCH_ON(h, h->stream, lds, "tm_learn+tm_scan+sp_overlap", kt_learn_scan_front[epl_slot(d)], grid, 256, d, h->tail_p, n_learn, n_scan, spec, in, h->sz.G, p, wmode);
            if (!wmode)
                for (int pass = 1; pass < d.sel_passes; ++pass) LAUNCH(h, "sp_select", k_sel_pass, h->sz.sel_blocks, RB, d, pass, p);
        } else {
            enqueue_sp_front(h, d.input_stage, 1, p, wmode, packed_input);
        }
        if (h->knob.step_split) {
            if (!emitted) enqueue_sp_back(h, d.input_stage, 1, p, 1, 0, false, wmode);
            const int lrn = learning ? 1 : 0;
            const int n_act = (d.k * d.KP + 255) / 256, n_rows = lrn ? d.k : 0;
            const int n_cls2 = lean2_classify_blocks(h, lrn);
            const int n_duty = h->sz.c256_blocks, n_clear = d.WPC * h->sz.c256_blocks;
            LAUNCH_ON(h, h->stream, 0, "tm_activate+tm_mid+sp_learn", k_act_mid_rows, n_act + 1 + n_cls2 + n_rows + n_duty + n_clear + h->sz.zero_blocks, 256,
                      d, p, d.k, n_act, lrn, n_cls2, d.input_stage, 1, n_rows, h->sz.G, 0, n_duty, n_clear, h->knob.lean2_order);
            h->tail_pending = true;
            h->tail_p = p;
        } else {
            enqueue_sp_back(h, d.input_stage, 1, p, 1, EMIT_ALL, false, wmode);
            enqueue_tm(h, d.k, learning ? 1 : 0, 1, p, d.input_stage, 1, true, -1, true);
        }
        h->step_host += 1;
        return launch_status(h->err);
    }
    flush_tail(h);
    return enqueue_step(h, h->d.input_stage, 1, learning ? 1 : 0, StepPlan{false, false, false}, packed_input);
}

extern "C" int htm_sp_step(htm_handle *h, const uint32_t *packed_input, int32_t learning) {
    if (!h || !packed_input) return HTM_ERR_ARGUMENT;
    if (h) flush_tail(h);
    REJECT_WHEN_AHEAD(h);
    if (!h->cfg.enable_sp) { h->err = "handle has no Spatial Pooler"; return HTM_ERR_STATE; }
    if (h->cfg.enable_tm) { h->err = "htm_sp_step: the handle also has a Temporal Memory; use htm_step"; return HTM_ERR_STATE; }
    HIPCHK(h, hipSetDevice(h->device));
    refresh_exchange_mode(h);
    int rc = close_open_phases(h);
    if (rc) return rc;
    rc = stage_input(h, packed_input);
    if (rc) return rc;
    const int p = (int)(h->step_host & 1);
    enqueue_sp_front(h, h->d.input_stage, 1, p, step_wmode(h));
    enqueue_sp_back(h, h->d.input_stage, 1, p, 0, EMIT_ALL, learning && !h->cfg.enable_tm, step_wmode(h));
    h->step_host += 1;
    return HTM_OK;
}

extern "C" int htm_sp_phase(htm_handle *h, int32_t phase, const void *data, int64_t count) {
    if (!h) return HTM_ERR_ARGUMENT;
    if (h) flush_tail(h);
    REJECT_WHEN_AHEAD(h);
    if (!h->cfg.enable_sp) { h->err = "handle has no Spatial Pooler"; return HTM_ERR_STATE; }
    if (h->world > 1) { h->err = "htm_sp_phase: not available on a column-sharded handle"; return HTM_ERR_STATE; }
    REFUSE_ON_VIEW(h, "htm_sp_phase");
    if (phase == HTM_SP_LEARN) weights_touched(h);
    HIPCHK(h, hipSetDevice(h->device));
    refresh_exchange_mode(h);
    Dev &d = h->d;
    const int p = (int)(h->step_host & 1);
    const int c256 = (d.C + 255) / 256;
    if (phase == HTM_SP_OVERLAP || phase == HTM_SP_BOOST || (phase == HTM_SP_SELECT && data))
        HIPCHK(h, hipMemsetAsync(d.hist0 + (size_t)p * HIST0_PAR, 0, (size_t)HIST0_PAR * 4, h->stream));
    switch (phase) {
        case HTM_SP_OVERLAP: {
            if (!data) return HTM_ERR_ARGUMENT;
            int rc = stage_input(h, (const uint32_t *)data);
            if (rc) return rc;
            LAUNCH(h, "sp_overlap", k_sp_overlap, h->sz.sp_blocks, RB, d, d.input_stage, 1, h->sz.G, p, p, 0, 0);
            break;
        }
        case HTM_SP_BOOST: {
            if (!data || count != d.C) { h->err = "htm_sp_phase(BOOST): need column_dim overlaps"; return HTM_ERR_ARGUMENT; }
            HIPCHK(h, hipMemcpyAsync(d.overlap[p], data, (size_t)d.C * 4, hipMemcpyHostToDevice, h->stream));
            HIPCHK(h, hipStreamSynchronize(h->stream));
            LAUNCH(h, "sp_keys", k_sp_keys, std::min((d.C + RB - 1) / RB, 256), RB, d, p, 1);
            break;
        }
        case HTM_SP_SELECT: {
            if (data) {
                if (count != d.C) { h->err = "htm_sp_phase(SELECT): need column_dim boosted overlaps"; return HTM_ERR_ARGUMENT; }
                HIPCHK(h, hipMemcpyAsync(d.boosted[p], data, (size_t)d.C * 8, hipMemcpyHostToDevice, h->stream));
                HIPCHK(h, hipStreamSynchronize(h->stream));
                LAUNCH(h, "sp_keys", k_sp_keys, std::min((d.C + RB - 1) / RB, 256), RB, d, p, 0);
            }
            for (int pass = 1; pass < d.sel_passes; ++pass) LAUNCH(h, "sp_select", k_sel_pass, h->sz.sel_blocks, RB, d, pass, p);
            enqueue_sp_back(h, d.input_stage, 1, p, 0, 0, false);
            break;
        }
        case HTM_SP_ACTIVE: {
            if ((!data && count) || count < 0 || count > d.k) { h->err = "htm_sp_phase(ACTIVE): at most active_columns columns"; return HTM_ERR_ARGUMENT; }
            std::vector<int> cols((const int *)data, (const int *)data + count);
            std::sort(cols.begin(), cols.end());
            for (int64_t i = 0; i < count; ++i)
                if (cols[i] < 0 || cols[i] >= d.C || (i && cols[i] == cols[i - 1])) { h->err = "htm_sp_phase(ACTIVE): bad column list"; return HTM_ERR_ARGUMENT; }
            if (count) HIPCHK(h, hipMemcpyAsync(d.active_cols[p], cols.data(), (size_t)count * 4, hipMemcpyHostToDevice, h->stream));
            HIPCHK(h, hipStreamSynchronize(h->stream));
            h->phase_active = (int)count;
            h->phase_open = true;
// ... 843 lines not shown
    HIPCHK(h, hipStreamSynchronize(h->stream));
    h->seg_hint = (int)(h->world > 1 ? own : total);
    if (h->seg_pinned) *h->seg_pinned = h->seg_hint;
    return HTM_OK;
}

extern "C" int htm_bank_upload(htm_handle *h, const uint32_t *host_inputs, int32_t n_inputs, uint32_t **device_bank) {
    if (!h || !host_inputs || n_inputs < 1 || !device_bank) return HTM_ERR_ARGUMENT;
    if (!h->cfg.enable_sp) { h->err = "handle has no Spatial Pooler"; return HTM_ERR_STATE; }
    Dev &d = h->d;
    HIPCHK(h, hipSetDevice(h->device));
    uint32_t *bank = nullptr;
    int rc = dalloc(h, &bank, (size_t)n_inputs * d.W);
    if (rc) return rc;
    const size_t words = (size_t)(d.I + 31) / 32;
    HIPCHK(h, hipMemcpy2DAsync(bank, (size_t)d.W * 4, host_inputs, words * 4, words * 4, (size_t)n_inputs,
                               hipMemcpyHostToDevice, h->stream));
    HIPCHK(h, hipStreamSynchronize(h->stream));
    *device_bank = bank;
    return HTM_OK;
}

static int read_counters(htm_handle *h, Counters *out) {
    HIPCHK(h, hipSetDevice(h->device));
    HIPCHK(h, hipStreamSynchronize(h->stream));
    HIPCHK(h, hipMemcpy(out, h->d.ctr, sizeof(Counters), hipMemcpyDeviceToHost));
    h->seg_hint = h->world > 1 ? out->L : out->S;
    if (h->seg_pinned) *h->seg_pinned = h->seg_hint;
    return 0;
}

extern "C" int htm_get_info(htm_handle *h, htm_info *out) {
    if (!h || !out) return HTM_ERR_ARGUMENT;
    if (h) flush_tail(h);
    Counters c;
    int rc = read_counters(h, &c);
    if (rc) return rc;
    const int q = (int)((h->step_host + 1) & 1);
    const int rows = h->world > 1 ? c.L : c.S;
    out->step_index = h->step_host;
    out->segments = c.S;
    out->local_segments = rows;
    out->matching_segments = 0;
    if (c.has_distal && rows > 0) {
        std::vector<uint32_t> bits(((size_t)rows + 31) / 32);
        HIPCHK(h, hipMemcpy(bits.data(), h->d.match_bits[q], bits.size() * 4, hipMemcpyDeviceToHost));
        for (int i = 0; i < rows; ++i) out->matching_segments += (bits[(size_t)i >> 5] >> (i & 31)) & 1u;
    }
    out->winner_cells = c.n_win[q];
    out->active_cells = c.n_active_cells;
    out->has_distal_state = c.has_distal;
    out->has_winner_cells = h->step_host > 0 ? c.has_winner[q] : 0;
    out->capacity_error = c.error;
    out->words_per_row = h->d.W;
    out->new_segment_requests = c.n_un;
    out->recycled_segments = c.n_un ? c.n_recycled : 0;
    out->appended_segments = c.n_un ? c.n_new : 0;
    out->work_items = c.n_work_last;
    out->select_fallbacks = c.sel_fallbacks;
    out->candidate_exact_steps = c.cand_exact;
    out->hot_select_steps = c.hot_selects;
    out->select_zoom_steps = c.sel_zooms;
    if (c.error) {
        h->err = std::string("capacity exhausted:") + ((c.error & 1) ? " segment pool (segment_capacity)" : "") +
                 ((c.error & 2) ? " synapse slots (segment_slots)" : "") + ((c.error & 4) ? " work list / growth staging" : "") +
                 ((c.error & 8) ? " dead-segment report (DEAD_CAP)" : "") +
                 ((c.error & 16) ? " (internal) block hand-off timed out in k_sp_emit" : "") +
                 ((c.error & 32) ? " (internal) the middle role's wait for the activation blocks timed out in k_act_mid_rows" : "") +
                 ((c.error & 64) ? " (not a capacity) htm_pack_columns met a column id outside this handle's input range" : "") +
                 ((c.error & 128) ? " (not a capacity) htm_tm_run met a list row with a repeated column id or one outside [0, column_dim): the results of its steps are invalid" : "");
        return HTM_ERR_CAPACITY;
    }
    return HTM_OK;
}

static inline int enc_flat(int enc, int K) { return K > 32 ? (enc >> 6) * K + (enc & 63) : (enc >> 5) * K + (enc & 31); }
static inline int flat_enc(int flat, int K) { return (flat / K) * (K > 32 ? 64 : 32) + (flat % K); }

extern "C" int64_t htm_read(htm_handle *h, int32_t field, void *dst, int64_t count) {
    if (!h || !dst) return HTM_ERR_ARGUMENT;
    if (h) flush_tail(h);
    const bool fixed_size = field == HTM_F_ACTIVE_COLUMN || field == HTM_F_OVERLAPS || field == HTM_F_BOOSTED || field == HTM_F_DUTY_CYCLE ||
                            field == HTM_F_CELL_ACTIVATION || field == HTM_F_CELL_PREDICTION || field == HTM_F_WINNER_WORDS ||
                            field == HTM_F_BURSTING || field == HTM_F_SEGCOUNT || field == HTM_F_CELL_MAX_JITTER;
    Counters c;
    memset(&c, 0, sizeof(c));
    int rc = 0;
    if (fixed_size) {
        HIPCHK(h, hipSetDevice(h->device));
        HIPCHK(h, hipStreamSynchronize(h->stream));
    } else {
        rc = read_counters(h, &c);
        if (rc) return rc;
    }
    Dev &d = h->d;
    const int q = (int)((h->step_host + 1) & 1);
    const int qs = h->phase_open ? (int)(h->step_host & 1) : q;
    const bool sp = h->cfg.enable_sp, tm = h->cfg.enable_tm;
    const int64_t C = d.C, K = d.K, S = h->world > 1 ? c.L : c.S, E = d.E, CW = (int64_t)d.C * d.WPC, KP = d.KP;
    auto need = [&](bool ok, int64_t n) -> int64_t {
        if (!ok) { h->err = "htm_read: field not available on this handle"; return HTM_ERR_STATE; }
        if (count < n) { h->err = "htm_read: buffer too small"; return HTM_ERR_ARGUMENT; }
        return n;
    };
    auto copy = [&](const void *src, int64_t n, size_t elem) -> int64_t {
        if (n > 0 && hipMemcpy(dst, src, (size_t)n * elem, hipMemcpyDeviceToHost) != hipSuccess) { h->err = "htm_read: hipMemcpy failed"; return HTM_ERR_HIP; }
        return n;
    };
    int64_t n;
    switch (field) {
        case HTM_F_ACTIVE_COLUMN: if ((n = need(true, d.k)) < 0) return n; return copy(d.active_cols[qs], n, 4);
        case HTM_F_OVERLAPS: REJECT_WHEN_AHEAD(h); if ((n = need(sp, C)) < 0) return n; return copy(d.overlap[qs], n, 4);
        case HTM_F_BOOSTED: REJECT_WHEN_AHEAD(h); if ((n = need(sp, C)) < 0) return n; return copy(d.boosted[qs], n, 8);
        case HTM_F_DUTY_CYCLE: REJECT_WHEN_AHEAD(h); if ((n = need(sp, C)) < 0) return n; return copy(d.duty, n, 4);
        case HTM_F_CELL_ACTIVATION: if ((n = need(tm, CW)) < 0) return n; return copy(d.act[q], n, 4);
        case HTM_F_CELL_PREDICTION: if ((n = need(tm, CW)) < 0) return n; return copy(d.pred[q], n, 4);
        case HTM_F_WINNER_WORDS: if ((n = need(tm, CW)) < 0) return n; return copy(d.win[q], n, 4);
        case HTM_F_BURSTING: if ((n = need(tm, d.k)) < 0) return n; return copy(d.bursting, n, 1);
        case HTM_F_SEG_NSYN: if ((n = need(tm, S)) < 0) return n; return copy(d.seg_nsyn, n, 4);
        case HTM_F_SEG_POTENTIAL:
        case HTM_F_MATCH_SEGMENT:
        case HTM_F_MATCH_INFO:
        case HTM_F_MATCH_JITTER: {
            if (!tm) { h->err = "htm_read: field not available on this handle"; return HTM_ERR_STATE; }
            if (field == HTM_F_SEG_POTENTIAL) {
                if ((n = need(true, S)) < 0) return n;
                if (S == 0) return 0;
                if (!c.has_distal) { memset(dst, 0, (size_t)S * 4); return S; }
                int *tmp = nullptr;
                if (hipMalloc((void **)&tmp, (size_t)S * 4) != hipSuccess) { h->err = "htm_read: hipMalloc failed"; return HTM_ERR_HIP; }
                hipLaunchKernelGGL(k_tm_potentials, dim3((unsigned)std::min<int64_t>((S * 8 + 255) / 256, 8192)), dim3(256), 0, h->stream, d, q, tmp, 0, (int)S);
                const bool ok = hipStreamSynchronize(h->stream) == hipSuccess && hipMemcpy(dst, tmp, (size_t)S * 4, hipMemcpyDeviceToHost) == hipSuccess;
                hipFree(tmp);
                if (!ok) { h->err = "htm_read: potentials kernel failed"; return HTM_ERR_HIP; }
                return S;
            }
            std::vector<uint32_t> bits(((size_t)S + 31) / 32, 0u);
            std::vector<uint32_t> info((size_t)S);
            std::vector<float> jit((size_t)S);
            if (S && c.has_distal && (hipMemcpy(bits.data(), d.match_bits[q], bits.size() * 4, hipMemcpyDeviceToHost) != hipSuccess ||
                                      hipMemcpy(info.data(), d.seg_info, (size_t)S * 4, hipMemcpyDeviceToHost) != hipSuccess ||
                                      hipMemcpy(jit.data(), d.seg_jit, (size_t)S * 4, hipMemcpyDeviceToHost) != hipSuccess)) { h->err = "htm_read: hipMemcpy failed"; return HTM_ERR_HIP; }
            auto is_matching = [&](int64_t i) { return (bits[(size_t)i >> 5] >> (i & 31)) & 1u; };
            int64_t m = 0;
            for (int64_t i = 0; i < S; ++i) m += is_matching(i);
            if ((n = need(true, m)) < 0) return n;
            m = 0;
            for (int64_t i = 0; i < S; ++i) {
                if (!is_matching(i)) continue;
                const uint32_t v = info[(size_t)i];
                if (field == HTM_F_MATCH_SEGMENT) ((int *)dst)[m] = (int)i;
                else if (field == HTM_F_MATCH_INFO) ((uint32_t *)dst)[m] = v & ~0x40000000u;
                else ((float *)dst)[m] = jit[(size_t)i];
                ++m;
            }
            return m;
        }
        case HTM_F_WINNER_CELL:
        case HTM_F_SEG_CELL: {
            const bool w = field == HTM_F_WINNER_CELL;
            if ((n = need(tm, w ? c.n_win[q] : S)) < 0) return n;
            if ((rc = (int)copy(w ? d.winners[q] : d.seg_cell, n, 4)) < 0) return rc;
            int *v = (int *)dst;
            for (int64_t i = 0; i < n; ++i) v[i] = enc_flat(v[i], (int)K);
            return n;
        }
        case HTM_F_SEG_PRESYN:
        case HTM_F_SEG_PERM: {
            if ((n = need(tm, S * E)) < 0) return n;
            std::vector<int> nsyn((size_t)S);
            if (S && hipMemcpy(nsyn.data(), d.seg_nsyn, (size_t)S * 4, hipMemcpyDeviceToHost) != hipSuccess) { h->err = "htm_read: hipMemcpy failed"; return HTM_ERR_HIP; }
            if ((rc = (int)copy(field == HTM_F_SEG_PRESYN ? (const void *)d.presyn : (const void *)d.sperm, n, 4)) < 0) return rc;
            for (int64_t s = 0; s < S; ++s)
                for (int64_t e = 0; e < E; ++e) {
                    const bool valid = e < nsyn[(size_t)s];
                    if (field == HTM_F_SEG_PRESYN) { int *v = (int *)dst + s * E + e; *v = valid ? enc_flat(*v & SYN_CELL, (int)K) : -1; }
                    else if (!valid) ((float *)dst)[s * E + e] = -1.0f;
                }
            return n;
        }
        case HTM_F_SEGCOUNT:
        case HTM_F_CELL_MAX_JITTER: {
            if ((n = need(tm, C * K)) < 0) return n;
            std::vector<uint32_t> tmp((size_t)C * KP);
            const void *src = field == HTM_F_SEGCOUNT ? (const void *)d.segcount : (const void *)d.cellmax[q];
            if (hipMemcpy(tmp.data(), src, tmp.size() * 4, hipMemcpyDeviceToHost) != hipSuccess) { h->err = "htm_read: hipMemcpy failed"; return HTM_ERR_HIP; }
            uint32_t *v = (uint32_t *)dst;
            for (int64_t col = 0; col < C; ++col)
                for (int64_t j = 0; j < K; ++j) v[col * K + j] = tmp[(size_t)col * KP + j];
            return n;
        }
        case HTM_F_SEG_GID: {
            if ((n = need(tm, S)) < 0) return n;
            if (d.seg_gid) return copy(d.seg_gid, n, 4);
            for (int64_t i = 0; i < n; ++i) ((int *)dst)[i] = (int)i;
            return n;
        }
// ... 879 lines not shown
```

bithtm_amd/csrc/htm_pipeline.h:

```cpp
#ifndef BITHTM_HTM_PIPELINE_H
#define BITHTM_HTM_PIPELINE_H

struct TraceScope {
    unsigned long long *t;
    __device__ TraceScope(const Dev &d, int slot) {
#if defined(BITHTM_LEARN_STAMPS) || defined(BITHTM_SCAN_STAMPS) || defined(BITHTM_EMIT_STAMPS) || defined(BITHTM_SHARD_STAMPS)
        t = nullptr;
        return;
#endif
        t = (d.trace && blockIdx.x < 4096 && d.ctr->step[slot >> 2] < d.trace_until) ? d.trace + ((size_t)slot * 4096 + blockIdx.x) * 2 : nullptr;
        if (t && threadIdx.x == 0) t[0] = wall_clock64();
    }
    __device__ ~TraceScope() { if (t && threadIdx.x == 0) t[1] = wall_clock64(); }
};

__global__ __launch_bounds__(256) void k_open_emit(Dev d, int p, int n_emit_blocks, int n_active) {
    TraceScope ts(d, 0 + 4 * p);
    if ((int)blockIdx.x < n_emit_blocks) {
        role_emit(d, p ^ 1, 1, 1, 0, blockIdx.x, n_emit_blocks, (EmitShared *)dyn_lds);
    } else {
        const int idx = ((int)blockIdx.x - n_emit_blocks) * tm_groups_per_block(d) + tm_group_of(d, threadIdx.x);
        const bool ok = idx < n_active;
        const int a = ok ? d.active_cols[p][idx] : 0;
        tm_activate_column(d, p, 1, ok, a, idx, tm_pred_words(d, p, ok, a));
// ... 72 lines not shown
    int b = blockIdx.x;
    if (b < n_act_blocks) {
        const int idx = b * tm_groups_per_block(d) + tm_group_of(d, threadIdx.x);
        const bool ok = idx < n_active;
        const int a = ok ? d.active_cols[p][idx] : 0;
        tm_activate_column(d, p, 1, ok, a, idx, tm_pred_words(d, p, ok, a));
        return;
    }
    b -= n_act_blocks;
    if (b < n_rows) {
        role_sp_row<256>(d, p, bank, n_inputs, 0, b, threadIdx.x);
        return;
    }
    b -= n_rows;
    const int c = b * 256 + (int)threadIdx.x;
    if (b < n_duty_blocks) {
        if (c < d.C) {
            float dc = d.duty[c] * d.mom;
            if ((d.colbits[p][c >> 5] >> (c & 31)) & 1u) dc = dc + d.dinc;
            d.duty[c] = dc;
        }
        return;
    }
    const int n_clear = (int)gridDim.x - n_act_blocks - n_rows - n_duty_blocks;
    for (int w = (b - n_duty_blocks) * 256 + (int)threadIdx.x; w < d.C * d.WPC; w += n_clear * 256) {
        const int cc = w >> (d.LK - 5);
        d.pred[p][w] = 0;
        if (!((d.colbits[p][cc >> 5] >> (cc & 31)) & 1u)) { d.act[p][w] = 0; d.win[p][w] = 0; }
    }
}

__global__ __launch_bounds__(256) void k_mid_overlap(Dev d, int p, int n_active, int want_winner, int learning, int n_cls,
                                                     const uint32_t *__restrict__ bank, int n_inputs, int G, int n_overlap_blocks) {
    TraceScope ts(d, 1 + 4 * p);
    int b = blockIdx.x;
    if (b <= n_cls) {
        role_mid<256>(d, p, n_active, want_winner, learning, b, n_cls);
        return;
    }
    b -= 1 + n_cls;
    if (b < n_overlap_blocks) {
        role_overlap<256>(d, bank, n_inputs, G, p, p ^ 1, 1, b, n_overlap_blocks, (uint32_t *)dyn_lds, 1);
        return;
    }
    b -= n_overlap_blocks;
    const int nz = (int)gridDim.x - 1 - n_cls - n_overlap_blocks;
    const int words4 = ((d.world > 1 ? d.ctr->L : d.ctr->S) + 127) >> 7;
    uint4 *mb = (uint4 *)d.match_bits[p];
    for (int i = b * 256 + (int)threadIdx.x; i < words4; i += nz * 256) mb[i] = make_uint4(0u, 0u, 0u, 0u);
}

__device__ __forceinline__ void fan_signal(const Dev &d, int p, int b) {
    asm volatile("s_waitcnt vmcnt(0)" ::: "memory");
    __syncthreads();
    if (threadIdx.x == 0)
        __hip_atomic_fetch_add(d.fan + (size_t)(p * FAN_COUNTERS + (b & (FAN_COUNTERS - 1))) * FAN_STRIDE, 1u, __ATOMIC_RELAXED, __HIP_MEMORY_SCOPE_AGENT);
}

__device__ __forceinline__ void fan_wait(const Dev &d, int p, uint32_t target) {
    if (threadIdx.x < 64) {
        for (int looks = 0;; ++looks) {
            uint32_t v = threadIdx.x < FAN_COUNTERS
                             ? __hip_atomic_load(d.fan + (size_t)(p * FAN_COUNTERS + (int)threadIdx.x) * FAN_STRIDE, __ATOMIC_RELAXED, __HIP_MEMORY_SCOPE_AGENT) : 0u;
            v = wave_sum(v);
            if (v >= target) break;
            if (looks >= (1 << 18)) {
                if (threadIdx.x == 0) atomicOr(&d.ctr->error, 32);
                break;
            }
#ifndef BITHTM_FAN_SLEEP
#define BITHTM_FAN_SLEEP 4
#endif
            __builtin_amdgcn_s_sleep(BITHTM_FAN_SLEEP);
        }
    }
    __syncthreads();
}

#ifndef BITHTM_LEAN2_WAVES
#define BITHTM_LEAN2_WAVES 8
#endif
__global__ __launch_bounds__(256, BITHTM_LEAN2_WAVES) void k_act_mid_rows(Dev d, int p, int n_active, int n_act_blocks, int learning, int n_cls,
                                                      const uint32_t *__restrict__ bank, int n_inputs, int n_rows, int G, int n_overlap_blocks,
                                                      int n_duty_blocks, int n_clear_blocks, int order) {
    TraceScope ts(d, 0 + 4 * p);
    int b = blockIdx.x;
    int role = 4;
#pragma unroll
    for (int i = 3; i >= 0 && role == 4; --i) {
        const int r = (order >> (4 * i)) & 15;
        const int n = r == 0 ? n_act_blocks : r == 1 ? 1 + n_cls : r == 2 ? n_rows : n_overlap_blocks;
        if (b < n) role = r; else b -= n;
    }
    if (role == 0) {
        const int idx = b * tm_groups_per_block(d) + tm_group_of(d, threadIdx.x);
        const bool ok = idx < n_active;
        const int a = ok ? d.active_cols[p][idx] : 0;
        tm_activate_column<true>(d, p, 1, ok, a, idx, tm_pred_words(d, p, ok, a));
        fan_signal(d, p, b);
        return;
    }
    if (role == 1) {
        role_mid<256>(d, p, n_active, 1, learning, b, n_cls, 1, [&]() { fan_wait(d, p, (uint32_t)n_act_blocks); });
        return;
    }
    if (role == 2) {
        if (n_overlap_blocks > 0) role_sp_row<256, true>(d, p, bank, n_inputs, 0, b, threadIdx.x);
        else role_sp_row<256>(d, p, bank, n_inputs, 0, b, threadIdx.x);
        return;
    }
    if (role == 3) {
        role_overlap<256>(d, bank, n_inputs, G, p, p ^ 1, 1, b, n_overlap_blocks, (uint32_t *)dyn_lds, 1, n_rows > 0 ? 2 : 1);
        return;
    }
    if (b < n_duty_blocks) {
        const int c = b * 256 + (int)threadIdx.x;
        if (c < d.C) {
            float dc = d.duty[c] * d.mom;
            if ((d.colbits[p][c >> 5] >> (c & 31)) & 1u) dc = dc + d.dinc;
            d.duty[c] = dc;
        }
        return;
    }
    b -= n_duty_blocks;
    if (b < n_clear_blocks) {
        for (int w = b * 256 + (int)threadIdx.x; w < d.C * d.WPC; w += n_clear_blocks * 256) {
            const int cc = w >> (d.LK - 5);
            d.pred[p][w] = 0;
            if (!((d.colbits[p][cc >> 5] >> (cc & 31)) & 1u)) { d.act[p][w] = 0; d.win[p][w] = 0; }
        }
        return;
    }
    b -= n_clear_blocks;
    const int nz = (int)gridDim.x - n_act_blocks - 1 - n_cls - n_rows - n_overlap_blocks - n_duty_blocks - n_clear_blocks;
    const int words4 = (d.ctr->S + 127) >> 7;
    uint4 *mb = (uint4 *)d.match_bits[p];
    for (int i = b * 256 + (int)threadIdx.x; i < words4; i += nz * 256) mb[i] = make_uint4(0u, 0u, 0u, 0u);
}

template <int EPL, int MINW, bool TAB = false>
__global__ __launch_bounds__(256, MINW) void k_learn_scan_emit(Dev d, int p, int n_emit_blocks, int n_learn_blocks, int n_scan_blocks, int n_spec) {
    TraceScope ts(d, 2 + 4 * p);
    constexpr bool LARGE = MINW < 6;
    static_assert(!(LARGE && TAB), "the streaming scan reads the cell words from memory");
    const bool dyn = LARGE && n_scan_blocks > 0;
    if (n_scan_blocks < 0) n_scan_blocks = -n_scan_blocks;
    if (blockIdx.x == gridDim.x - 1 && threadIdx.x < FAN_COUNTERS) d.fan[(size_t)(p * FAN_COUNTERS + (int)threadIdx.x) * FAN_STRIDE] = 0u;
    int b = blockIdx.x, scan_blk;
    if (b < n_emit_blocks) {
        role_emit(d, p ^ 1, 1, 1, 0, b, n_emit_blocks, (EmitShared *)dyn_lds, 1);
        if (!dyn) return;
        scan_blk = -1 - b;
    } else if (b < n_emit_blocks + n_learn_blocks) {
        role_learn<EPL, 256, true>(d, p, b - n_emit_blocks, n_learn_blocks, (LearnShared<EPL, 256> *)dyn_lds);
        if (!dyn) return;
        scan_blk = -1 - b;
    } else {
        scan_blk = b - n_emit_blocks - n_learn_blocks;
    }
    if (LARGE) role_scan<256, true, true, false, true>(d, p, scan_blk, n_scan_blocks, dyn ? n_emit_blocks + n_learn_blocks : 0, (uint32_t *)dyn_lds);
    else role_scan<256, true, false, TAB>(d, p, scan_blk, n_scan_blocks, n_spec, (uint32_t *)dyn_lds);
}

template <int EPL>
__global__ __launch_bounds__(256, 6) void k_learn_scan_tail(Dev d, int p, int n_learn_blocks, int n_scan_blocks, int n_spec,
                                                            const uint32_t *__restrict__ bank, int n_inputs, int G, int wmode, int n_rows) {
    int b = blockIdx.x;
    if (blockIdx.x == gridDim.x - 1 && threadIdx.x < FAN_COUNTERS) d.fan[(size_t)(p * FAN_COUNTERS + (int)threadIdx.x) * FAN_STRIDE] = 0u;
    if (b < n_learn_blocks) {
        role_learn<EPL, 256, true>(d, p, b, n_learn_blocks, (LearnShared<EPL, 256> *)dyn_lds);
        return;
    }
    b -= n_learn_blocks;
    if (b < n_scan_blocks) {
        role_scan<256, true, false, false>(d, p, b, n_scan_blocks, n_spec, (uint32_t *)dyn_lds);
        return;
    }
    b -= n_scan_blocks;
    if (n_rows > 0) role_sp_row<256>(d, p, bank, n_inputs, 0, b, threadIdx.x);
    else role_overlap<256>(d, bank, n_inputs, G, p, p ^ 1, 1, b, (int)gridDim.x - n_learn_blocks - n_scan_blocks, (uint32_t *)dyn_lds, wmode);
}

template <int EPL>
__global__ __launch_bounds__(256, 6) void k_learn_scan_front(Dev d, int p_prev, int n_learn_blocks, int n_scan_blocks, int n_spec,
                                                             PackedInputArg in, int G, int p, int wmode) {
    int b = blockIdx.x;
    if (blockIdx.x == gridDim.x - 1 && threadIdx.x < FAN_COUNTERS) d.fan[(size_t)(p_prev * FAN_COUNTERS + (int)threadIdx.x) * FAN_STRIDE] = 0u;
    if (b < n_learn_blocks) {
        role_learn<EPL, 256, true>(d, p_prev, b, n_learn_blocks, (LearnShared<EPL, 256> *)dyn_lds);
        return;
    }
    b -= n_learn_blocks;
    if (b < n_scan_blocks) {
        role_scan<256, true, false, false>(d, p_prev, b, n_scan_blocks, n_spec, (uint32_t *)dyn_lds);
        return;
// ... 14 lines not shown
```

bithtm_amd/csrc/htm_sp_kernels.h:

```cpp
#ifndef BITHTM_HTM_SP_KERNELS_H
#define BITHTM_HTM_SP_KERNELS_H


__global__ __launch_bounds__(256) void k_sp_build_mask(Dev d, int row_begin, int row_count) {
    const int wave = (blockIdx.x * blockDim.x + threadIdx.x) >> 6;
    const int nwaves = (gridDim.x * blockDim.x) >> 6;
    const int lane = lane_id();
    const int chunks = d.Ipad >> 6;
    for (long long t = wave; t < (long long)row_count * chunks; t += nwaves) {
        int row = row_begin + (int)(t / chunks), ch = (int)(t % chunks);
        int i = ch * 64 + lane;
        bool conn = (i < d.I) && (d.perm[(size_t)row * d.Ipad + i] >= d.sp_thr);
        u64 m = __ballot(conn);
        if (lane == 0) *(u64 *)&d.mask[(size_t)row * d.W + ch * 2] = m;
    }
}

#ifdef BITHTM_OVERLAP_STAMPS
#define OV_STAMP(i) do { if (d.trace && wmode && threadIdx.x == 0 && blk < 512) d.trace[(size_t)3 * 8192 + (size_t)blk * 8 + (i)] = wall_clock64(); } while (0)
#else
#define OV_STAMP(i) do { } while (0)
#endif
template <int BS>
__device__ __forceinline__ void role_overlap(const Dev &d, const uint32_t *__restrict__ bank, int n_inputs, int G,
                                             int p, int sp, int step_offset, int blk, int nblk, uint32_t *h, int wmode = 0, int fold = 0) {
    const int gtid = blk * BS + threadIdx.x;
    const int nthreads = nblk * BS;
    uint32_t *ghist = d.hist + sp * SEL_MAX_PASSES * SEL_BINS;
    OV_STAMP(0);
    if (gtid == 0) d.ctr->emit_epoch += 1;
    const uint4 *in4 = (const uint4 *)bank;
    if (n_inputs > 1) in4 = (const uint4 *)(bank + (size_t)((d.ctr->step[p] + (uint32_t)step_offset) % (uint32_t)n_inputs) * d.W);
    const uint4 *mask4 = (const uint4 *)d.mask;
    const int lane = lane_id();
    const int rpw = 64 / G, sub = lane / G, l = lane % G;
    const int wave = gtid >> 6, nwaves = nthreads >> 6;
    constexpr int U = 4;
    const bool spread = G == 8;
    const int first_row0 = d.c0 + wave * rpw * U;
    uint4 m[U];
    float dty_first = 0.f;
    uint32_t cbw_first = 0u;
#pragma unroll
    for (int u = 0; u < U; ++u) {
        const int row = first_row0 + u * rpw + sub;
        m[u] = (row < d.c1 && l < d.W4) ? mask4[(uint32_t)row * (uint32_t)d.W4 + (uint32_t)l] : make_uint4(0, 0, 0, 0);
    }
    if (spread) {
        const int row = first_row0 + (l & 3) * rpw + sub;
        dty_first = (l < U && row < d.c1) ? d.duty[row] : 0.f;
        if (fold) cbw_first = (l < U && row < d.c1) ? d.colbits[p][row >> 5] : 0u;
    }
    for (int i = gtid; i < (d.sel_passes - 1) * SEL_BINS; i += nthreads) ghist[SEL_BINS + i] = 0;
    for (int i = threadIdx.x; i < SEL_BINS; i += BS) h[i] = 0;
    if (gtid == 0) {
        d.ctr->sel_pass_prefix[sp][0] = 0;
        d.ctr->sel_pass_krem[sp][0] = (uint32_t)d.sel_k;
    }
    const uint32_t wbase = wmode ? d.ctr->sel_win[sp] : 0u;
    lds_barrier();
    OV_STAMP(1);
    static_assert(WIN_BINS <= SEL_BINS - SEL_COARSE, "the runs' sums live behind the window's bins in the LDS histogram");
    uint32_t *hc = h + SEL_BINS - SEL_COARSE;
    auto finish_row = [&](bool owner, int row, int cn, float duty, uint32_t cbw) {
        u64 key = 0;
        if (owner && fold) {
            duty = duty * d.mom;
            if ((cbw >> (row & 31)) & 1u) {
                if (fold == 2) owner = false;
                else duty = duty + d.dinc;
            }
            if (owner) d.duty[row] = duty;
        }
        if (owner) {
            d.overlap[sp][row] = cn;
            const float f = htm_exp_f32(d.coef * duty);
            const double bo = (double)f * (double)cn;
            d.boosted[sp][row] = bo;
            key = select_key(bo);
            d.key[sp][row] = key;
        }
        const uint32_t bin = wmode ? win_bin(key, wbase) : (uint32_t)(key >> sel_shift(0));
        if (owner && (!wmode || bin != 0u)) {
            atomicAdd(&h[bin], 1u);
            if (wmode) atomicAdd(&hc[bin >> 6], 1u);
        }
    };
    for (int row0 = first_row0; row0 < d.c1; row0 += nwaves * rpw * U) {
        const bool first = row0 == first_row0;
        int cnt[U];
        float dty = dty_first;
        uint32_t cbw = cbw_first;
#pragma unroll
        for (int u = 0; u < U; ++u) cnt[u] = 0;
        if (!first && spread) {
            const int row = row0 + (l & 3) * rpw + sub;
            dty = (l < U && row < d.c1) ? d.duty[row] : 0.f;
            if (fold) cbw = (l < U && row < d.c1) ? d.colbits[p][row >> 5] : 0u;
        }
        for (int j = l; j < d.W4; j += G) {
            if (!(first && j == l)) {
#pragma unroll
                for (int u = 0; u < U; ++u) {
                    const int row = row0 + u * rpw + sub;
                    m[u] = row < d.c1 ? mask4[(uint32_t)row * (uint32_t)d.W4 + (uint32_t)j] : make_uint4(0, 0, 0, 0);
                }
            }
            const uint4 x = in4[j];
#pragma unroll
            for (int u = 0; u < U; ++u)
                cnt[u] += __popc(m[u].x & x.x) + __popc(m[u].y & x.y) + __popc(m[u].z & x.z) + __popc(m[u].w & x.w);
        }
        OV_STAMP(2);
        if (spread) {
            int mine = 0;
#pragma unroll
            for (int u = 0; u < U; ++u) {
                const int cn = group8_sum_all(cnt[u]);
                if (l == u) mine = cn;
            }
            const int row = row0 + (l & 3) * rpw + sub;
            finish_row(l < U && row < d.c1, row, mine, dty, cbw);
        } else {
#pragma unroll
            for (int u = 0; u < U; ++u) {
                int cn = cnt[u];
                for (int o = G >> 1; o > 0; o >>= 1) cn += __shfl_xor(cn, o);
                const int row = row0 + u * rpw + sub;
                const bool mine = l == 0 && row < d.c1;
                finish_row(mine, row, cn, mine ? d.duty[row] : 0.f, (fold && mine) ? d.colbits[p][row >> 5] : 0u);
            }
        }
    }
    OV_STAMP(3);
    lds_barrier();
    OV_STAMP(4);
    uint32_t *g0 = d.hist0 + (size_t)sp * HIST0_PAR + (size_t)(blk & (HIST_REP - 1)) * SEL_BINS;
    uint32_t *gc = d.hist0 + (size_t)sp * HIST0_PAR + HIST0_FINE + (size_t)(blk & (COARSE_REP - 1)) * COARSE_STRIDE;
    const int n_fine = wmode ? SEL_BINS - SEL_COARSE : SEL_BINS;
    {
        constexpr int PER = SEL_BINS / BS;
        uint32_t v[PER];
#pragma unroll
        for (int k = 0; k < PER; ++k) v[k] = h[threadIdx.x + k * BS];
#pragma unroll
        for (int k = 0; k < PER; ++k) {
            const int i = threadIdx.x + k * BS;
            if (v[k] && i < n_fine) atomicAdd(&g0[i], v[k]);
        }
    }
    if (wmode && threadIdx.x < SEL_COARSE && hc[threadIdx.x]) atomicAdd(&gc[threadIdx.x], hc[threadIdx.x]);
    OV_STAMP(5);
}

__global__ __launch_bounds__(RB) void k_sp_overlap(Dev d, const uint32_t *__restrict__ bank, int n_inputs, int G, int p, int sp, int step_offset, int wmode) {
    __shared__ uint32_t h[SEL_BINS];
    role_overlap<RB>(d, bank, n_inputs, G, p, sp, step_offset, blockIdx.x, gridDim.x, h, wmode);
}

#define ARG_INPUT_WORDS 64
struct PackedInputArg { uint32_t w[ARG_INPUT_WORDS]; };
__global__ __launch_bounds__(RB) void k_sp_overlap_arg(Dev d, PackedInputArg in, int G, int p, int wmode) {
    __shared__ uint32_t h[SEL_BINS];
    __shared__ __attribute__((aligned(16))) uint32_t s_in[ARG_INPUT_WORDS];
    if (threadIdx.x < ARG_INPUT_WORDS) {
        const uint32_t v = threadIdx.x < d.W ? in.w[threadIdx.x] : 0u;
        s_in[threadIdx.x] = v;
        if (blockIdx.x == 0 && threadIdx.x < d.W) d.input_stage[threadIdx.x] = v;
    }
    __syncthreads();
    role_overlap<RB>(d, s_in, 1, G, p, p, 0, blockIdx.x, gridDim.x, h, wmode);
}

template <int BS>
__device__ __forceinline__ void sel_resolve(const Dev &d, int sp, int prev, uint32_t *h, uint32_t *s_wave,
                                            u64 *out_prefix, uint32_t *out_krem, u64 *s_res_prefix, uint32_t *s_res_krem) {
    const int tid = threadIdx.x, lane = lane_id(), wv = tid >> 6;
    const int shift = sel_shift(prev), nb = 1 << sel_bits(prev);
    const u64 prefix = d.ctr->sel_pass_prefix[sp][prev];
    const uint32_t krem = d.ctr->sel_pass_krem[sp][prev];
    const uint32_t *gh = d.hist + (sp * SEL_MAX_PASSES + prev) * SEL_BINS;
    constexpr int PER = SEL_BINS / BS;
    static_assert(PER % 4 == 0, "16-byte histogram accesses");
    {
        uint4 v[PER / 4];
#pragma unroll
        for (int j = 0; j < PER / 4; ++j) {
            const int b = 4 * (j * BS + tid);
            v[j] = (prev > 0 && b < nb) ? *(const uint4 *)(gh + b) : make_uint4(0, 0, 0, 0);
        }
        if (prev == 0) {
            const uint32_t *g0 = d.hist0 + (size_t)sp * HIST0_PAR;
            for (int r = 0; r < HIST_REP; ++r)
#pragma unroll
                for (int j = 0; j < PER / 4; ++j) {
                    const uint4 a = *(const uint4 *)(g0 + (size_t)r * SEL_BINS + 4 * (j * BS + tid));
                    v[j].x += a.x; v[j].y += a.y; v[j].z += a.z; v[j].w += a.w;
                }
        }
#pragma unroll
        for (int j = 0; j < PER / 4; ++j) *(uint4 *)(h + 4 * (j * BS + tid)) = v[j];
    }
    __syncthreads();
    uint32_t cs = 0;
#pragma unroll
    for (int j = 0; j < PER / 4; ++j) {
        const uint4 v = *(const uint4 *)(h + tid * PER + 4 * j);
        cs += v.x + v.y + v.z + v.w;
    }
    const uint32_t pre = wave_incl_scan(cs);
    const uint32_t wtot = (uint32_t)__builtin_amdgcn_readlane((int)pre, 63);
    if (lane == 0) s_wave[wv] = wtot;
    __syncthreads();
    uint32_t above = wtot - pre;
    for (int w = wv + 1; w < BS / 64; ++w) above += s_wave[w];
    if (above < krem && krem <= above + cs) {
        for (int b = min((tid + 1) * PER, nb) - 1; b >= tid * PER; --b) {
            const uint32_t hb = h[b];
            if (above + hb >= krem) {
                *s_res_prefix = prefix | ((u64)b << shift);
                *s_res_krem = krem - above;
                break;
            }
            above += hb;
        }
    }
    __syncthreads();
    *out_prefix = *s_res_prefix;
    *out_krem = *s_res_krem;
}

struct SelShared { uint32_t h[SEL_BINS]; uint32_t wave[16]; u64 prefix; uint32_t krem; };

template <int BS>
__device__ __forceinline__ void role_sel_pass(const Dev &d, int pass, int sp, int blk, int nblk, SelShared *sh) {
// ... 851 lines not shown
    }
    if (b == 0 && tid == 0 && !d.act[0]) d.ctr->step[p ^ 1] = d.ctr->step[p] + 1;
    EMIT_STAMP(5);
    if (!tm_here && !local) return;
    __syncthreads();
    const int n_sel = s_n;
    if (local) {
        double *r_boost = (double *)d.send;
        uint32_t *r_col = (uint32_t *)(d.send + (size_t)d.cand_cap * 8), *r_win = r_col + d.cand_cap, *r_unacc = r_win + d.cand_cap;
        const int has_distal = d.ctr->has_distal;
        const uint32_t step = d.ctr->step[p];
        constexpr int CPP = 4;
        for (int i0 = 0; i0 < n_sel; i0 += 8 * CPP) {
            int a[CPP];
            bool ok[CPP];
            ColumnLoads l[CPP];
            double bo[CPP];
#pragma unroll
            for (int u = 0; u < CPP; ++u) {
                const int i = i0 + u * 8 + (tid >> 5);
                ok[u] = i < n_sel;
                a[u] = ok[u] ? s_col[i] : d.c0;
                l[u] = tm_column_loads(d, p, ok[u], a[u], has_distal);
                bo[u] = d.boosted[p][a[u]];
            }
#pragma unroll
            for (int u = 0; u < CPP; ++u) {
                const ColumnWords w = tm_column_compute(d, 1, ok[u], a[u], ok[u] ? s_predw[a[u] - cbase] : 0u, l[u], has_distal, step);
                const int pos = first_pos + i0 + u * 8 + (tid >> 5);
                if (ok[u] && (lane & 31) == 0) {
                    r_boost[pos] = bo[u];
                    r_col[pos] = (uint32_t)a[u] | (w.burst ? 0x80000000u : 0u);
                    r_win[pos] = w.winner;
                    r_unacc[pos] = w.unacc;
                }
            }
        }
        for (int i = d.sel_k + b * 256 + tid; i < d.cand_cap; i += nblk * 256) ((u64 *)r_boost)[i] = CAND_PAD;
        if (b == 0) {
            uint32_t *r_dead = r_unacc + d.cand_cap;
            const int n = min(d.dead_list[0], DEAD_CAP);
            if (tid == 0) {
                r_dead[0] = (uint32_t)n;
                uint32_t *r_n = (uint32_t *)(d.send + shard_record_count_offset(d.cand_cap));
                r_n[0] = (uint32_t)d.sel_k;
                r_n[1] = CAND_HOT_NONE;
                if (fused && wmode) d.ctr->cand_exact += 1;
            }
            for (int j = tid; j < n; j += 256) r_dead[1 + j] = (uint32_t)d.dead_list[1 + j];
        }
        return;
    }
    for (int i0 = 0; i0 < n_sel; i0 += tm_groups_per_block(d)) {
        const int i = i0 + tm_group_of(d, tid);
        const bool ok = i < n_sel;
        const int a = ok ? s_col[i] : 0;
        tm_activate_column(d, p, want_winner, ok, a, first_pos + i, d.WPC == 1 ? (u64)(ok ? s_predw[a - cbase] : 0u) : tm_pred_words(d, p, ok, a));
    }
}

__global__ __launch_bounds__(256) void k_sp_emit(Dev d, int p, int want_winner, int fused, int mode, int wmode, int n_emit_blocks) {
    __shared__ EmitShared sh;
    if ((int)blockIdx.x >= n_emit_blocks) {
        const int nb = (int)gridDim.x - n_emit_blocks;
        for (int c = ((int)blockIdx.x - n_emit_blocks) * 256 + (int)threadIdx.x; c < d.C * d.WPC; c += nb * 256) {
            d.act[p][c] = 0;
            d.win[p][c] = 0;
            d.pred[p][c] = 0;
            if (c < d.colwords) d.colbits[p][c] = 0;
        }
        return;
    }
    role_emit(d, p, want_winner, fused, mode, blockIdx.x, n_emit_blocks, &sh, wmode);
}

__global__ __launch_bounds__(256) void k_sp_learn(Dev d, const uint32_t *__restrict__ bank, int n_inputs, int p) {
    const uint32_t *in = bank + (size_t)(d.ctr->step[p] % (uint32_t)n_inputs) * d.W;
    const int row = d.active_cols[p][blockIdx.x];
    double *prow = d.perm + (size_t)row * d.Ipad;
    uint32_t *mrow = d.mask + (size_t)row * d.W;
    for (int i0 = 0; i0 < d.Ipad; i0 += 256) {
        int i = i0 + threadIdx.x;
        bool conn = false;
        if (i < d.I) {
            bool on = (in[i >> 5] >> (i & 31)) & 1u;
            double v = prow[i] + (on ? d.sp_don : d.sp_doff);
            prow[i] = v;
            conn = v >= d.sp_thr;
        }
        u64 m = __ballot(conn);
        if (lane_id() == 0 && i < d.Ipad) *(u64 *)&mrow[i >> 5] = m;
    }
}

__global__ __launch_bounds__(RB) void k_sp_keys(Dev d, int p, int from_overlap) {
    __shared__ uint32_t h[SEL_BINS];
    const int gtid = blockIdx.x * RB + threadIdx.x, nthreads = gridDim.x * RB;
    uint32_t *ghist = d.hist + p * SEL_MAX_PASSES * SEL_BINS;
    if (gtid == 0) {
        d.ctr->emit_epoch += 1;
        d.ctr->sel_pass_prefix[p][0] = 0;
        d.ctr->sel_pass_krem[p][0] = (uint32_t)d.sel_k;
    }
    for (int i = gtid; i < (d.sel_passes - 1) * SEL_BINS; i += nthreads) ghist[SEL_BINS + i] = 0;
    for (int i = threadIdx.x; i < SEL_BINS; i += RB) h[i] = 0;
    __syncthreads();
    for (int c = d.sel_lo + gtid; c < d.sel_hi; c += nthreads) {
        double bo;
        if (from_overlap) {
            const float f = htm_exp_f32(d.coef * d.duty[c]);
            bo = (double)f * (double)d.overlap[p][c];
            d.boosted[p][c] = bo;
        } else {
            bo = d.boosted[p][c];
        }
        const u64 key = select_key(bo);
        d.key[p][c] = key;
        atomicAdd(&h[(uint32_t)(key >> sel_shift(0))], 1u);
    }
    __syncthreads();
    uint32_t *g0 = d.hist0 + (size_t)p * HIST0_PAR + (size_t)(blockIdx.x & (HIST_REP - 1)) * SEL_BINS;
    for (int i = threadIdx.x; i < SEL_BINS; i += RB)
        if (h[i]) atomicAdd(&g0[i], h[i]);
}

__global__ __launch_bounds__(256) void k_sp_list_bits(Dev d, int p, int n, int pass) {
    const int i = blockIdx.x * 256 + threadIdx.x;
    if (pass == 0) { if (i < d.colwords) d.colbits[p][i] = 0; return; }
    if (i < n) { const int c = d.active_cols[p][i]; atomicOr(&d.colbits[p][c >> 5], 1u << (c & 31)); }
}

__global__ __launch_bounds__(256) void k_sp_duty_list(Dev d, int p, int n, int pass) {
    const int i = blockIdx.x * 256 + threadIdx.x;
    if (pass == 0) { if (i < d.C) d.duty[i] = d.duty[i] * d.mom; return; }
    if (i < n) { const int c = d.active_cols[p][i]; d.duty[c] = d.duty[c] + d.dinc; }
}

__global__ void k_sp_commit(Dev d, int p) { d.ctr->step[p ^ 1] = d.ctr->step[p] + 1; }

__global__ __launch_bounds__(RB) void k_shard_overlap(Dev d, const uint32_t *__restrict__ bank, int n_inputs, int G, int p, int wmode, int front) {
    __shared__ uint32_t h[SEL_BINS];
    role_overlap<RB>(d, bank, n_inputs, G, p, front ? p ^ 1 : p, front ? 1 : 0, blockIdx.x, gridDim.x, h, wmode);
}

struct BlockSelLds { uint32_t *h, *s_wave, *s_out, *s_cnt; u64 *s_or, *s_and; unsigned long long *trace; };
#ifdef BITHTM_SHARD_STAMPS
#define SHARD_STAMP(i) do { if (d.trace && blockIdx.x == 0 && threadIdx.x == 0) d.trace[i] = wall_clock64(); } while (0)
#define SEL_STAMP(i) do { if (L.trace && blockIdx.x == 0 && threadIdx.x == 0) L.trace[i] = wall_clock64(); } while (0)
#else
#define SHARD_STAMP(i) do { } while (0)
#define SEL_STAMP(i) do { } while (0)
#endif

template <int KPT>
__device__ __forceinline__ void block_select_regs(const u64 (&kreg)[KPT], uint32_t vmask, uint32_t k, uint32_t base, int low_zero,
                                                  const BlockSelLds &L, u64 *T_out, uint32_t *r_out, bool *missed, bool h_zeroed = false) {
    const int tid = threadIdx.x, lane = lane_id();
    uint32_t *h = L.h;
    u64 P = 0;
    uint32_t krem = k;
    bool done = false;
    u64 T = 0;
    int top_start = 64, top0 = 64;
    bool outside = false;
    {
        if (!h_zeroed) {
            for (int i = tid; i < SEL_BINS; i += 1024) h[i] = 0;
            if (tid == 0) { L.s_cnt[0] = 0; L.s_out[0] = 0; *L.s_or = 0; *L.s_and = ~0ull; }
            lds_barrier();
        }
        SEL_STAMP(8);
#pragma unroll
        for (int j = 0; j < KPT; ++j) {
            const uint32_t bin = win_bin(kreg[j], base);
// ... 392 lines not shown
```

bithtm_amd/csrc/htm_tm_kernels.h:

```cpp
#ifndef BITHTM_HTM_TM_KERNELS_H
#define BITHTM_HTM_TM_KERNELS_H


__global__ __launch_bounds__(256) void k_tm_load_active(Dev d, int p, const int *cols, int n) {
    for (int c = blockIdx.x * 256 + threadIdx.x; c < d.C * d.WPC; c += gridDim.x * 256) {
        d.act[p][c] = 0;
        d.pred[p][c] = 0;
        d.win[p][c] = 0;
        if (c < n) d.active_cols[p][c] = cols[c];
        if (c < d.colwords) d.colbits[p][c] = 0;
    }
}

__global__ __launch_bounds__(256) void k_tm_activate(Dev d, int p, int n_active, int want_winner) {
    const int idx = blockIdx.x * tm_groups_per_block(d) + tm_group_of(d, threadIdx.x);
    const bool ok = idx < n_active;
    const int a = ok ? d.active_cols[p][idx] : 0;
    if (ok && (threadIdx.x & (d.KP - 1)) == 0) atomicOr(&d.colbits[p][a >> 5], 1u << (a & 31));
    tm_activate_column(d, p, want_winner, ok, a, idx, tm_pred_words(d, p, ok, a));
}

__global__ __launch_bounds__(256) void k_tm_ext_winners(Dev d, int p, const int *cols, const uint32_t *winw, const uint32_t *unacc, int n, int pass) {
    const int i = blockIdx.x * 256 + threadIdx.x;
    if (pass == 0) { for (int c = i; c < d.C * d.WPC; c += gridDim.x * 256) d.win[p][c] = 0; return; }
// ... 23 lines not shown
        const uint32_t cells = wave_sum(cnt);
        if (lane_id() == 0 && cells) atomicAdd(&d.ctr->n_active_cells, (int)cells);
    }
}

__device__ __forceinline__ bool col_is_local(const Dev &d, int cell) { const int col = cell >> d.LK; return col >= d.c0 && col < d.c1; }

__device__ __forceinline__ int seg_gid_of(const Dev &d, int row) { return d.seg_gid ? d.seg_gid[row] : row; }

__device__ __forceinline__ void tm_bind_segment(const Dev &d, int seg, int cell, bool recycled, int pos) {
    if (recycled) atomicSub(&d.segcount[d.seg_cell[seg]], 1);
    d.seg_cell[seg] = cell;
    d.seg_nsyn[seg] = (int)SEG_BUSY;
    atomicAdd(&d.segcount[cell], 1);
    if (pos < d.work_cap) d.work[pos] = (uint32_t)seg; else atomicOr(&d.ctr->error, 4);
}

__device__ __forceinline__ void shard_bind(const Dev &d, int p, int gid, int cell, bool recycled, int grown, int pass) {
    Counters *c = d.ctr;
    const bool to_me = col_is_local(d, cell);
    const int old_row = recycled ? d.g2l[gid] : -1;
    if (pass == 0) {
        const bool alive = grown >= d.match_thr;
        if (recycled && alive) { atomicAnd(&d.dead_bits[gid >> 5], ~(1u << (gid & 31))); recyc_add(d, gid >> 10, -1); }
        if (!recycled && !alive) { atomicOr(&d.dead_bits[gid >> 5], 1u << (gid & 31)); recyc_add(d, gid >> 10, 1); }
        if (old_row >= 0) {
            atomicSub(&d.segcount[d.seg_cell[old_row]], 1);
            if (!to_me) {
                d.seg_gid[old_row] = -1;
                d.seg_nsyn[old_row] = 0;
                d.g2l[gid] = -1;
                d.lfree[atomicAdd(&c->n_lfree, 1)] = old_row;
            }
        }
        return;
    }
    if (!to_me) return;
    int row = old_row;
    if (row < 0) {
        const int top = atomicSub(&c->n_lfree, 1) - 1;
        if (top >= 0) {
            row = d.lfree[top];
        } else {
            atomicAdd(&c->n_lfree, 1);
            row = atomicAdd(&c->L, 1);
        }
        if (row >= d.Lcap) { atomicOr(&c->error, 1); return; }
        d.seg_gid[row] = gid;
        d.g2l[gid] = row;
    }
    d.seg_cell[row] = cell;
    d.seg_nsyn[row] = (int)SEG_BUSY;
    atomicAdd(&d.segcount[cell], 1);
    const int pos = atomicAdd(&c->n_work[p], 1);
    if (pos < d.work_cap) d.work[pos] = (uint32_t)row; else atomicOr(&c->error, 4);
}

#ifdef BITHTM_ROWS_STAMPS
#define ROW_STAMP(i) do { if (d.trace && t == 0 && ri < 1024) d.trace[(size_t)7 * 8192 + (size_t)ri * 8 + (i)] = wall_clock64(); } while (0)
#else
#define ROW_STAMP(i) do { } while (0)
#endif
template <int TPR, bool OWN = false>
__device__ __forceinline__ void role_sp_row(const Dev &d, int p, const uint32_t *__restrict__ bank, int n_inputs, int ahead, int ri, int t) {
    ROW_STAMP(0);
    const uint32_t step = ahead ? d.ctr->step[p ^ 1] + 1u : d.ctr->step[p];
    const uint32_t *in = bank + (size_t)(step % (uint32_t)n_inputs) * d.W;
    const uint32_t *in_next = bank + (size_t)((step + 1u) % (uint32_t)n_inputs) * d.W;
    const int row = d.active_cols[p][ri];
    if (row < d.c0 || row >= d.c1) return;
    ROW_STAMP(1);
    double *prow = d.perm + (size_t)row * d.Ipad;
    uint32_t *mrow = d.mask + (size_t)row * d.W;
    float duty0 = 0.f;
    uint32_t wbase = 0u;
    if (OWN && t == 0) {
        duty0 = d.duty[row];
        wbase = d.ctr->sel_win[p ^ 1];
    }
    int own_cn = 0;
    for (int i0 = 0; i0 < d.Ipad; i0 += 2 * TPR) {
        const int e0 = i0 + 2 * t;
        bool c0 = false, c1 = false;
        if (e0 < d.Ipad) {
            double2 v = *(double2 *)(prow + e0);
            const uint32_t bits = in[e0 >> 5] >> (e0 & 31);
            const uint32_t nbits = OWN ? in_next[e0 >> 5] >> (e0 & 31) : 0u;
            if (e0 < d.I) { v.x = v.x + ((bits & 1u) ? d.sp_don : d.sp_doff); c0 = v.x >= d.sp_thr; }
            if (e0 + 1 < d.I) { v.y = v.y + ((bits & 2u) ? d.sp_don : d.sp_doff); c1 = v.y >= d.sp_thr; }
            if (OWN) own_cn += (int)(c0 && (nbits & 1u)) + (int)(c1 && (nbits & 2u));
            if (i0 == 0) ROW_STAMP(2); else ROW_STAMP(4);
            {
                typedef unsigned int u32x4 __attribute__((ext_vector_type(4)));
                union { double2 d2; u32x4 u4; } cvt;
                cvt.d2 = v;
                double *dst = prow + e0;
                asm volatile("global_store_dwordx4 %0, %1, off sc0 sc1\n\ts_nop 1" ::"v"(dst), "v"(cvt.u4) : "memory");
            }
        }
        const u64 b0 = __ballot(c0), b1 = __ballot(c1);
        const int base = i0 + 2 * (t & ~63);
        if (lane_id() == 0 && base < d.Ipad) {
            u64 *mw = (u64 *)&mrow[base >> 5];
            const u64 m0 = spread32((uint32_t)b0) | (spread32((uint32_t)b1) << 1);
            const u64 m1 = spread32((uint32_t)(b0 >> 32)) | (spread32((uint32_t)(b1 >> 32)) << 1);
            mw[0] = m0;
            mw[1] = m1;
        }
        if (i0 == 0) ROW_STAMP(3); else ROW_STAMP(5);
    }
    if (OWN) {
        __shared__ int s_own[TPR / 64];
        own_cn = (int)wave_sum((uint32_t)own_cn);
        if (lane_id() == 0) s_own[t >> 6] = own_cn;
        __syncthreads();
        if (t == 0) {
            int cn = 0;
#pragma unroll
            for (int wv = 0; wv < TPR / 64; ++wv) cn += s_own[wv];
            const int sp = p ^ 1;
            float dc = duty0 * d.mom;
            dc = dc + d.dinc;
            d.duty[row] = dc;
            d.overlap[sp][row] = cn;
            const float f = htm_exp_f32(d.coef * dc);
            const double bo = (double)f * (double)cn;
            d.boosted[sp][row] = bo;
            const u64 key = select_key(bo);
            d.key[sp][row] = key;
            const uint32_t bin = win_bin(key, wbase);
            if (bin != 0u) {
                atomicAdd(d.hist0 + (size_t)sp * HIST0_PAR + (size_t)(ri & (HIST_REP - 1)) * SEL_BINS + bin, 1u);
                atomicAdd(d.hist0 + (size_t)sp * HIST0_PAR + HIST0_FINE + (size_t)(ri & (COARSE_REP - 1)) * COARSE_STRIDE + (bin >> 6), 1u);
            }
        }
    }
}

template <typename T>
__device__ __forceinline__ T ld_agent(const T *ptr, int same_launch) {
    return same_launch ? __hip_atomic_load(ptr, __ATOMIC_RELAXED, __HIP_MEMORY_SCOPE_AGENT) : *ptr;
}
struct NoWait { __device__ __forceinline__ void operator()() const {} };
template <int BS, typename Wait = NoWait>
__device__ __forceinline__ void role_mid(const Dev &d, int p, int n_active, int want_winner, int learning, int blk, int n_cls, int same_launch = 0,
                                         Wait wait = Wait()) {
    Counters *c = d.ctr;
    __shared__ int s_words[BS];
    __shared__ uint32_t s_bits[BS];
    __shared__ int s_nwords;
    if (blk > 0) {
        if (!learning || !c->has_distal) return;
        const int q = p ^ 1;
        const int n = d.world > 1 ? c->L : c->S;
        bool waited = false;
        auto wait_once = [&]() { if (!waited) { wait(); waited = true; } };
        auto gather = [&](int seg, bool &cand, bool &punish, int &cell) {
            const uint32_t info = d.seg_info[seg];
            cell = d.seg_cell[seg];
            const float jit = d.seg_jit[seg];
            const int cw = cell >> 5, cb = cell & 31, col = cell >> d.LK;
            const bool on_col = (d.colbits[p][col >> 5] >> (col & 31)) & 1u;
            const bool unpred = !((d.pred[q][cw] >> cb) & 1u);
            const bool best = fabsf(jit - __uint_as_float(d.cellmax[q][cell])) < d.eps;
            cand = ((info >> 31) || (unpred && best)) && (on_col || !same_launch);
            punish = d.punish ? (d.punish[cw] >> cb) & 1u : !on_col;
        };
        auto decide = [&](bool cand, int cell) {
            return cand && ((ld_agent(&d.win[p][cell >> 5], same_launch) >> (cell & 31)) & 1u);
        };
        if (n <= (d.cls_rows_max >= 0 ? d.cls_rows_max : (same_launch ? 2 : 8) * n_cls * BS)) {
            for (int i0 = (blk - 1) * BS; i0 < n; i0 += n_cls * BS) {
                const int seg = i0 + (int)threadIdx.x;
                bool cand = false, punish = false;
                int cell = 0;
                if (seg < n && ((d.match_bits[q][seg >> 5] >> (seg & 31)) & 1u)) gather(seg, cand, punish, cell);
                wait_once();
                const bool learn = decide(cand, cell);
                if (learn || punish) d.seg_nsyn[seg] |= (int)SEG_BUSY;
                const u64 ml = __ballot(learn), mp = __ballot(punish);
                const int n_l = __popcll(ml), n_p = __popcll(mp);
                if (n_l + n_p == 0) continue;
                int base = 0;
                if (lane_id() == 0) base = atomicAdd(&c->n_work[p], n_l + n_p);
                base = wave_read(base, 0);
                if (learn) {
                    const int pos = base + __popcll(ml & lanemask_lt());
                    if (pos < d.work_cap) d.work[pos] = (uint32_t)seg; else atomicOr(&c->error, 4);
                }
                if (punish) {
// ... 1099 lines not shown
```

include/bithtm_hip.h:

```cpp
#ifndef BITHTM_HIP_H
#define BITHTM_HIP_H

#include <stddef.h>
#include <stdint.h>

#ifdef __cplusplus
extern "C" {
#endif

#define BITHTM_ABI_VERSION 4

typedef struct htm_handle htm_handle;

typedef enum htm_status {
    HTM_OK = 0,
    HTM_ERR_ARGUMENT = -1,
    HTM_ERR_HIP = -2,
    HTM_ERR_CAPACITY = -3,
    HTM_ERR_STATE = -4
} htm_status;

typedef struct htm_config {
    uint32_t struct_bytes;
    int32_t device;
    int32_t input_dim;
    int32_t column_dim;
    int32_t cell_dim;
    int32_t active_columns;
    int32_t enable_sp;
    int32_t enable_tm;
    double sp_permanence_threshold;
    double sp_delta_on;
    double sp_delta_off;
    float boost_coefficient;
    float duty_momentum;
    float duty_increment;
    double tm_learn_active;
    double tm_learn_inactive;
    double tm_punish_active;
    double tm_punish_inactive;
    int32_t tm_learn_prune;
    int32_t tm_punish_prune;
    float tm_permanence_initial;
    float tm_permanence_threshold;
    int32_t segment_activation_threshold;
    int32_t segment_matching_threshold;
    int32_t segment_sampling_synapses;
    int32_t segment_capacity;
    int32_t segment_capacity_local;
    int32_t segment_slots;
    uint32_t seed;
    int32_t shard_rank;
    int32_t shard_world;
    int32_t use_caller_stream;
    void *stream;
} htm_config;

typedef struct htm_info {
    int64_t step_index;
    int32_t segments;
    int32_t local_segments;
    int32_t matching_segments;
    int32_t winner_cells;
    int32_t active_cells;
    int32_t has_distal_state;
    int32_t has_winner_cells;
    int32_t capacity_error;
    int32_t words_per_row;
    int32_t new_segment_requests;
    int32_t recycled_segments;
    int32_t appended_segments;
    int32_t work_items;
    int32_t select_fallbacks;
    int32_t candidate_exact_steps;
    int32_t hot_select_steps;
    int32_t select_zoom_steps;
} htm_info;

typedef enum htm_field {
    HTM_F_ACTIVE_COLUMN = 1,
    HTM_F_OVERLAPS = 2,
    HTM_F_BOOSTED = 3,
    HTM_F_DUTY_CYCLE = 4,
    HTM_F_CELL_ACTIVATION = 5,
    HTM_F_CELL_PREDICTION = 6,
    HTM_F_WINNER_WORDS = 7,
    HTM_F_BURSTING = 8,
    HTM_F_WINNER_CELL = 9,
    HTM_F_SEG_CELL = 10,
    HTM_F_SEG_NSYN = 11,
    HTM_F_SEG_PRESYN = 12,
    HTM_F_SEG_PERM = 13,
    HTM_F_SEGCOUNT = 14,
    HTM_F_SEG_POTENTIAL = 15,
    HTM_F_MATCH_SEGMENT = 16,
    HTM_F_MATCH_INFO = 17,
    HTM_F_MATCH_JITTER = 18,
    HTM_F_CELL_MAX_JITTER = 19,
    HTM_F_SEG_GID = 20
} htm_field;

int htm_create(const htm_config *config, htm_handle **out);
void htm_destroy(htm_handle *h);
const char *htm_last_error(const htm_handle *h);
int htm_abi_version(void);

int htm_sp_set_permanence(htm_handle *h, const double *rows, int32_t row_begin, int32_t row_count);

int htm_set_epsilon(htm_handle *h, float epsilon);
int htm_sp_get_permanence(htm_handle *h, double *rows, int32_t row_begin, int32_t row_count);

int htm_step(htm_handle *h, const uint32_t *packed_input, int32_t learning);
int htm_sp_step(htm_handle *h, const uint32_t *packed_input, int32_t learning);
int htm_tm_step(htm_handle *h, const int32_t *active_column, int32_t n, int32_t learning,
                int32_t return_winner_cell);

int htm_tm_update(htm_handle *h, const int32_t *columns, const uint32_t *winner_words, const uint32_t *unaccounted_words,
                  int32_t n, const uint32_t *punish_words);
int htm_tm_scan(htm_handle *h, const uint32_t *active_words);

typedef enum htm_sp_phase_id {
    HTM_SP_OVERLAP = 1,
    HTM_SP_BOOST = 2,
    HTM_SP_SELECT = 3,
    HTM_SP_ACTIVE = 4,
    HTM_SP_LEARN = 5,
    HTM_SP_DUTY = 6,
    HTM_SP_COMMIT = 7
} htm_sp_phase_id;
int htm_sp_phase(htm_handle *h, int32_t phase, const void *data, int64_t count);

int htm_run(htm_handle *h, const uint32_t *device_inputs, int32_t n_inputs, int32_t n_steps,
            int32_t learning, int32_t use_graph);
#define HTM_RUN_GRAPH 1
#define HTM_RUN_NO_PIPELINE 2
#define HTM_RUN_CONTINUE 4

int htm_prepare(htm_handle *h, const uint32_t *device_inputs, int32_t n_inputs, int32_t n_steps,
                int32_t learning, int32_t use_graph);

#define HTM_PLAN_GRAPH 1
#define HTM_PLAN_PIPELINED 2
#define HTM_PLAN_LEAN 4
#define HTM_PLAN_SCAN_LARGE 8
int htm_run_plan(htm_handle *h, int32_t n_steps, int32_t use_graph);

typedef struct htm_step_record {
    int32_t active_columns;
    int32_t bursting_columns;
    int32_t predicted_columns_before;
    int32_t predicted_columns;
    int32_t active_cells;
    int32_t winner_cells;
    int32_t segments;
    int32_t new_segments;
} htm_step_record;

typedef struct htm_run_record {
    uint32_t struct_bytes;
    htm_step_record *records;
    int32_t *active_column;
    uint32_t *column_prediction;
} htm_run_record;

int htm_run_recorded(htm_handle *h, const uint32_t *device_inputs, int32_t n_inputs, int32_t n_steps, int32_t learning,
                     int32_t use_graph, const htm_run_record *rec);
int htm_prepare_recorded(htm_handle *h, const uint32_t *device_inputs, int32_t n_inputs, int32_t n_steps, int32_t learning,
                         int32_t use_graph);
int htm_reset(htm_handle *h);
int htm_set_run_resets(htm_handle *h, const uint32_t *device_bits, int32_t n_inputs);
int htm_predicted_input(htm_handle *h, int32_t *host_dst);
int htm_set_run_predicted_input(htm_handle *h, int32_t *device_votes);

int htm_graph_count(htm_handle *h);

int htm_bank_upload(htm_handle *h, const uint32_t *host_inputs, int32_t n_inputs, uint32_t **device_bank);

int64_t htm_shard_record_bytes(htm_handle *h);
int htm_shard_begin(htm_handle *h, const uint32_t *device_inputs, int32_t n_inputs, const uint32_t *packed_input,
                    int32_t learning, void *send_device);
int htm_shard_finish(htm_handle *h, const void *recv_device, int32_t learning);

// ... 65 lines not shown
```

Baseline: 42120 timesteps/s.

## Compute SP overlap from transposed byte-plane mask over nonzero input bytes

```diff
diff --git a/bithtm_amd/_lib.py b/bithtm_amd/_lib.py
--- a/bithtm_amd/_lib.py
+++ b/bithtm_amd/_lib.py
@@ -51,6 +51,8 @@
 F_WINNER_WORDS, F_BURSTING, F_WINNER_CELL, F_SEG_CELL, F_SEG_NSYN, F_SEG_PRESYN, F_SEG_PERM = 7, 8, 9, 10, 11, 12, 13
 F_SEGCOUNT, F_SEG_POTENTIAL, F_MATCH_SEGMENT, F_MATCH_INFO, F_MATCH_JITTER, F_CELL_MAX_JITTER = 14, 15, 16, 17, 18, 19
 F_SEG_GID = 20
+F_SP_MASK = 21
+F_SP_MASK_PLANES = 22
 PLAN_GRAPH, PLAN_PIPELINED, PLAN_LEAN, PLAN_SCAN_LARGE = 1, 2, 4, 8
 SP_OVERLAP, SP_BOOST, SP_SELECT, SP_ACTIVE, SP_LEARN, SP_DUTY, SP_COMMIT = 1, 2, 3, 4, 5, 6, 7
 
diff --git a/bithtm_amd/csrc/htm_dev.h b/bithtm_amd/csrc/htm_dev.h
--- a/bithtm_amd/csrc/htm_dev.h
+++ b/bithtm_amd/csrc/htm_dev.h
@@ -82,6 +82,7 @@
 
 struct Dev {
     int I, W, W4, Ipad, C, K, k, E, Scap, work_cap, sel_passes, colwords, low_zero, cand_d, cand_pairwise, cand_others, cand_speculate, cand_take_all, cand_zoom, poll_delay;
+    int Cp;
     int win_offset;
     int cls_rows_max;
     int LK, KP, WPC;
@@ -100,6 +101,7 @@
     uint32_t seed;
     double *perm;
     uint32_t *mask;
+    uint8_t *mask_planes;
     float *duty;
     int *overlap[2];
     double *boosted[2];
@@ -302,6 +304,19 @@
     return x;
 }
 
+__device__ __forceinline__ void planes_store_changed(const Dev &d, int row, int byte0, u64 oldw, u64 neww) {
+#ifdef BITHTM_PLANES_STORE_ALL
+    const u64 diff = ~0ull;
+#else
+    const u64 diff = oldw ^ neww;
+#endif
+    if (diff == 0ull) return;
+    uint8_t *pl = d.mask_planes + (size_t)byte0 * (size_t)d.Cp + (size_t)row;
+#pragma unroll
+    for (int b = 0; b < 8; ++b)
+        if ((diff >> (8 * b)) & 0xFFull) pl[(size_t)b * (size_t)d.Cp] = (uint8_t)(neww >> (8 * b));
+}
+
 __device__ __forceinline__ uint32_t cell_mask(int K) { return K >= 32 ? 0xFFFFFFFFu : ((1u << K) - 1u); }
 __device__ __forceinline__ u64 cell_mask64(int K) { return K >= 64 ? ~0ull : ((1ull << K) - 1ull); }
 __device__ __forceinline__ uint32_t cell_mask_word(int K, int h) { return cell_mask(K - 32 * h); }
diff --git a/bithtm_amd/csrc/htm_engine.hip b/bithtm_amd/csrc/htm_engine.hip
--- a/bithtm_amd/csrc/htm_engine.hip
+++ b/bithtm_amd/csrc/htm_engine.hip
@@ -43,6 +43,7 @@
     uint32_t trace_until;
     int lean, lean2_classify, lean2_order, step_split, fuse_tm, shard_window, step_window, tail_rows, scan_large, scan_large_above, scan_dyn;
     int defer_tail, shared_scan, shared_members;
+    int overlap_planes, planes_dense;
     int lean_overlap, lean_learn, lean_learn_large, lean_scan, lean_scan_large, scan_blocks, sel_launch_digits;
     int cand_d, cand_pairwise, cls_rows_max, win_offset, cand_zoom, cand_speculate, cand_take_all, poll_delay, cand_others;
 };
@@ -50,7 +51,7 @@
 struct Sizes {
     int G;
     int sp_blocks, sel_blocks, c256_blocks, s1024_blocks, scan_blocks, zero_blocks, cus;
-    int lean_learn_blocks, lean_learn_blocks_large, lean_scan_blocks, lean_scan_blocks_large, lean_overlap_blocks, lean2_classify_blocks;
+    int lean_learn_blocks, lean_learn_blocks_large, lean_scan_blocks, lean_scan_blocks_large, lean_overlap_blocks, lean2_overlap_blocks, plane_above, lean2_classify_blocks;
     int lean_resident_large;
     bool emit_fits, emit_fits_open;
     bool emit_fits_lean;
@@ -434,13 +435,14 @@
 static void enqueue_lean(htm_handle *h, int p, int learning, const uint32_t *bank, int n_inputs, StepPlan plan) {
     Dev &d = h->d;
     const int n_act = (d.k * d.KP + 255) / 256, n_rows = learning ? d.k : 0;
-    const int n_cls = learning ? kClassifyBlocks : 0, n_ov = plan.next_sp ? h->sz.lean_overlap_blocks : 0;
+    const int n_cls = learning ? kClassifyBlocks : 0;
+    const int n_ov = plan.next_sp ? (h->knob.lean == 2 ? h->sz.lean2_overlap_blocks : h->sz.lean_overlap_blocks) : 0;
     if (h->knob.lean == 2) {
         const int n_cls2 = lean2_classify_blocks(h, learning);
         const int n_duty = n_ov ? 0 : h->sz.c256_blocks, n_clear = d.WPC * h->sz.c256_blocks;
         LAUNCH_ON(h, h->stream, (size_t)SEL_BINS * 4, "tm_activate+tm_mid+sp_learn+sp_overlap", k_act_mid_rows,
                   n_act + 1 + n_cls2 + n_rows + n_ov + n_duty + n_clear + h->sz.zero_blocks, 256, d, p, d.k, n_act, learning, n_cls2, bank, n_inputs, n_rows, h->sz.G, n_ov,
-                  n_duty, n_clear, h->knob.lean2_order);
+                  n_duty, n_clear, h->knob.lean2_order, h->sz.plane_above);
     } else {
         LAUNCH(h, "tm_activate+sp_learn", k_act_rows, n_act + n_rows + (1 + d.WPC) * h->sz.c256_blocks, 256, d, p, d.k, n_act, bank, n_inputs, n_rows, h->sz.c256_blocks);
         LAUNCH_ON(h, h->stream, (size_t)SEL_BINS * 4, "tm_mid+sp_overlap", k_mid_overlap, 1 + n_cls + n_ov + h->sz.zero_blocks, 256, d, p, d.k, 1, learning, n_cls,
@@ -585,6 +587,7 @@
     if (cfg->enable_sp) {
         rc |= dalloc_weights(h, &d.perm, C * d.Ipad);
         rc |= dalloc_weights(h, &d.mask, C * d.W);
+        rc |= dalloc_weights(h, &d.mask_planes, (size_t)4 * d.W * d.Cp);
     }
     if (cfg->enable_tm) {
         const size_t S = d.Lcap, E = d.E, KP = d.KP;
@@ -708,6 +711,8 @@
     k.shared_scan = env_flag("BITHTM_SHARED_SCAN", 0);
     k.shared_members = env_int("BITHTM_SHARED_SCAN_MEMBERS", 0, 0);
     k.lean_overlap = env_int("BITHTM_LEAN_OVERLAP", 0, 1);
+    k.overlap_planes = env_flag("BITHTM_OVERLAP_PLANES", 1);
+    k.planes_dense = env_int("BITHTM_OVERLAP_PLANES_DENSE", 50, 0, 100);
     k.lean_learn = env_int("BITHTM_LEAN_LEARN", 0, 1);
     k.lean_learn_large = env_int("BITHTM_LEAN_LEARN_LARGE", 0, 1);
     k.lean_scan = env_int("BITHTM_LEAN_SCAN", 0, 1);
@@ -741,6 +746,8 @@
     if (z.scan_blocks > 256) z.scan_blocks = (z.scan_blocks + 255) & ~255;
     z.zero_blocks = std::max(1, std::min((d.Lcap / 128 + 4095) / 4096, 1024));
     z.lean_overlap_blocks = k.lean_overlap ? k.lean_overlap : z.sp_blocks * (RB / 256);
+    z.plane_above = k.overlap_planes && 4 * d.W <= PLANE_MAX_BYTES ? 4 * d.W * k.planes_dense / 100 : -1;
+    z.lean2_overlap_blocks = k.lean_overlap || z.plane_above < 0 ? z.lean_overlap_blocks : std::max(1, std::min(z.lean_overlap_blocks, (d.Cp / 4 + 255) / 256));
     z.lean_learn_blocks = k.lean_learn ? k.lean_learn : 512;
     z.lean_learn_blocks_large = k.lean_learn_large ? k.lean_learn_large : k.lean_learn ? z.lean_learn_blocks : 768;
     z.lean_scan_blocks = k.lean_scan ? k.lean_scan : (z.scan_blocks > 512 ? std::max(256, (z.scan_blocks * 3 / 8 + 255) & ~255) : z.scan_blocks);
@@ -842,6 +849,7 @@
     d.W4 = d.W / 4;
     d.Ipad = d.W * 32;
     d.C = cfg->column_dim;
+    d.Cp = (d.C + 3) & ~3;
     d.world = world;
     d.c0 = h->rank * (d.C / world);
     d.c1 = d.c0 + d.C / world;
@@ -1081,6 +1089,8 @@
     const long long waves = (long long)row_count * (d.Ipad / 64);
     const int blocks = (int)std::min<long long>((waves + 3) / 4, 8192);
     hipLaunchKernelGGL(k_sp_build_mask, dim3(blocks), dim3(256), 0, h->stream, d, row_begin, row_count);
+    const int pblocks = (int)std::min<long long>(((long long)row_count * d.W + 255) / 256, 8192);
+    hipLaunchKernelGGL(k_mask_planes_rebuild, dim3(pblocks), dim3(256), 0, h->stream, d, row_begin, row_count);
     HIPCHK(h, hipStreamSynchronize(h->stream));
     return HTM_OK;
 }
@@ -1166,7 +1176,7 @@
             const int n_cls2 = lean2_classify_blocks(h, lrn);
             const int n_duty = h->sz.c256_blocks, n_clear = d.WPC * h->sz.c256_blocks;
             LAUNCH_ON(h, h->stream, 0, "tm_activate+tm_mid+sp_learn", k_act_mid_rows, n_act + 1 + n_cls2 + n_rows + n_duty + n_clear + h->sz.zero_blocks, 256,
-                      d, p, d.k, n_act, lrn, n_cls2, d.input_stage, 1, n_rows, h->sz.G, 0, n_duty, n_clear, h->knob.lean2_order);
+                      d, p, d.k, n_act, lrn, n_cls2, d.input_stage, 1, n_rows, h->sz.G, 0, n_duty, n_clear, h->knob.lean2_order, -1);
             h->tail_pending = true;
             h->tail_p = p;
         } else {
@@ -2176,7 +2186,8 @@
     if (h) flush_tail(h);
     const bool fixed_size = field == HTM_F_ACTIVE_COLUMN || field == HTM_F_OVERLAPS || field == HTM_F_BOOSTED || field == HTM_F_DUTY_CYCLE ||
                             field == HTM_F_CELL_ACTIVATION || field == HTM_F_CELL_PREDICTION || field == HTM_F_WINNER_WORDS ||
-                            field == HTM_F_BURSTING || field == HTM_F_SEGCOUNT || field == HTM_F_CELL_MAX_JITTER;
+                            field == HTM_F_BURSTING || field == HTM_F_SEGCOUNT || field == HTM_F_CELL_MAX_JITTER ||
+                            field == HTM_F_SP_MASK || field == HTM_F_SP_MASK_PLANES;
     Counters c;
     memset(&c, 0, sizeof(c));
     int rc = 0;
@@ -2207,6 +2218,8 @@
         case HTM_F_OVERLAPS: REJECT_WHEN_AHEAD(h); if ((n = need(sp, C)) < 0) return n; return copy(d.overlap[qs], n, 4);
         case HTM_F_BOOSTED: REJECT_WHEN_AHEAD(h); if ((n = need(sp, C)) < 0) return n; return copy(d.boosted[qs], n, 8);
         case HTM_F_DUTY_CYCLE: REJECT_WHEN_AHEAD(h); if ((n = need(sp, C)) < 0) return n; return copy(d.duty, n, 4);
+        case HTM_F_SP_MASK: REJECT_WHEN_AHEAD(h); if ((n = need(sp, C * d.W)) < 0) return n; return copy(d.mask, n, 4);
+        case HTM_F_SP_MASK_PLANES: REJECT_WHEN_AHEAD(h); if ((n = need(sp, (int64_t)4 * d.W * d.Cp)) < 0) return n; return copy(d.mask_planes, n, 1);
         case HTM_F_CELL_ACTIVATION: if ((n = need(tm, CW)) < 0) return n; return copy(d.act[q], n, 4);
         case HTM_F_CELL_PREDICTION: if ((n = need(tm, CW)) < 0) return n; return copy(d.pred[q], n, 4);
         case HTM_F_WINNER_WORDS: if ((n = need(tm, CW)) < 0) return n; return copy(d.win[q], n, 4);
diff --git a/bithtm_amd/csrc/htm_pipeline.h b/bithtm_amd/csrc/htm_pipeline.h
--- a/bithtm_amd/csrc/htm_pipeline.h
+++ b/bithtm_amd/csrc/htm_pipeline.h
@@ -178,7 +178,7 @@
 #endif
 __global__ __launch_bounds__(256, BITHTM_LEAN2_WAVES) void k_act_mid_rows(Dev d, int p, int n_active, int n_act_blocks, int learning, int n_cls,
                                                       const uint32_t *__restrict__ bank, int n_inputs, int n_rows, int G, int n_overlap_blocks,
-                                                      int n_duty_blocks, int n_clear_blocks, int order) {
+                                                      int n_duty_blocks, int n_clear_blocks, int order, int plane_above) {
     TraceScope ts(d, 0 + 4 * p);
     int b = blockIdx.x;
     int role = 4;
@@ -206,7 +206,9 @@
         return;
     }
     if (role == 3) {
-        role_overlap<256>(d, bank, n_inputs, G, p, p ^ 1, 1, b, n_overlap_blocks, (uint32_t *)dyn_lds, 1, n_rows > 0 ? 2 : 1);
+        const int fold = n_rows > 0 ? 2 : 1;
+        if (plane_above < 0 || !role_overlap_planes<256>(d, bank, n_inputs, p, p ^ 1, 1, b, n_overlap_blocks, (uint32_t *)dyn_lds, 1, fold, plane_above))
+            role_overlap<256>(d, bank, n_inputs, G, p, p ^ 1, 1, b, n_overlap_blocks, (uint32_t *)dyn_lds, 1, fold);
         return;
     }
     if (b < n_duty_blocks) {
diff --git a/bithtm_amd/csrc/htm_sp_kernels.h b/bithtm_amd/csrc/htm_sp_kernels.h
--- a/bithtm_amd/csrc/htm_sp_kernels.h
+++ b/bithtm_amd/csrc/htm_sp_kernels.h
@@ -16,11 +16,66 @@
     }
 }
 
+__global__ __launch_bounds__(256) void k_mask_planes_rebuild(Dev d, int row_begin, int row_count) {
+    const long long n = (long long)row_count * d.W;
+    for (long long t = (long long)blockIdx.x * blockDim.x + threadIdx.x; t < n; t += (long long)gridDim.x * blockDim.x) {
+        const int row = row_begin + (int)(t % row_count), w = (int)(t / row_count);
+        const uint32_t m = d.mask[(size_t)row * d.W + w];
+#pragma unroll
+        for (int b = 0; b < 4; ++b) d.mask_planes[(size_t)(4 * w + b) * (size_t)d.Cp + (size_t)row] = (uint8_t)(m >> (8 * b));
+    }
+}
+
 #ifdef BITHTM_OVERLAP_STAMPS
 #define OV_STAMP(i) do { if (d.trace && wmode && threadIdx.x == 0 && blk < 512) d.trace[(size_t)3 * 8192 + (size_t)blk * 8 + (i)] = wall_clock64(); } while (0)
 #else
 #define OV_STAMP(i) do { } while (0)
 #endif
+__device__ __forceinline__ void overlap_finish_row(const Dev &d, int sp, int wmode, int fold, uint32_t wbase, uint32_t *h, uint32_t *hc,
+                                                   bool owner, int row, int cn, float duty, uint32_t cbw) {
+    u64 key = 0;
+    if (owner && fold) {
+        duty = duty * d.mom;
+        if ((cbw >> (row & 31)) & 1u) {
+            if (fold == 2) owner = false;
+            else duty = duty + d.dinc;
+        }
+        if (owner) d.duty[row] = duty;
+    }
+    if (owner) {
+        d.overlap[sp][row] = cn;
+        const float f = htm_exp_f32(d.coef * duty);
+        const double bo = (double)f * (double)cn;
+        d.boosted[sp][row] = bo;
+        key = select_key(bo);
+        d.key[sp][row] = key;
+    }
+    const uint32_t bin = wmode ? win_bin(key, wbase) : (uint32_t)(key >> sel_shift(0));
+    if (owner && (!wmode || bin != 0u)) {
+        atomicAdd(&h[bin], 1u);
+        if (wmode) atomicAdd(&hc[bin >> 6], 1u);
+    }
+}
+
+template <int BS>
+__device__ __forceinline__ void overlap_flush(const Dev &d, int sp, int wmode, int blk, const uint32_t *h, const uint32_t *hc) {
+    uint32_t *g0 = d.hist0 + (size_t)sp * HIST0_PAR + (size_t)(blk & (HIST_REP - 1)) * SEL_BINS;
+    uint32_t *gc = d.hist0 + (size_t)sp * HIST0_PAR + HIST0_FINE + (size_t)(blk & (COARSE_REP - 1)) * COARSE_STRIDE;
+    const int n_fine = wmode ? SEL_BINS - SEL_COARSE : SEL_BINS;
+    {
+        constexpr int PER = SEL_BINS / BS;
+        uint32_t v[PER];
+#pragma unroll
+        for (int k = 0; k < PER; ++k) v[k] = h[threadIdx.x + k * BS];
+#pragma unroll
+        for (int k = 0; k < PER; ++k) {
+            const int i = threadIdx.x + k * BS;
+            if (v[k] && i < n_fine) atomicAdd(&g0[i], v[k]);
+        }
+    }
+    if (wmode && threadIdx.x < SEL_COARSE && hc[threadIdx.x]) atomicAdd(&gc[threadIdx.x], hc[threadIdx.x]);
+}
+
 template <int BS>
 __device__ __forceinline__ void role_overlap(const Dev &d, const uint32_t *__restrict__ bank, int n_inputs, int G,
                                              int p, int sp, int step_offset, int blk, int nblk, uint32_t *h, int wmode = 0, int fold = 0) {
@@ -62,30 +117,7 @@
     OV_STAMP(1);
     static_assert(WIN_BINS <= SEL_BINS - SEL_COARSE, "the runs' sums live behind the window's bins in the LDS histogram");
     uint32_t *hc = h + SEL_BINS - SEL_COARSE;
-    auto finish_row = [&](bool owner, int row, int cn, float duty, uint32_t cbw) {
-        u64 key = 0;
-        if (owner && fold) {
-            duty = duty * d.mom;
-            if ((cbw >> (row & 31)) & 1u) {
-                if (fold == 2) owner = false;
-                else duty = duty + d.dinc;
-            }
-            if (owner) d.duty[row] = duty;
-        }
-        if (owner) {
-            d.overlap[sp][row] = cn;
-            const float f = htm_exp_f32(d.coef * duty);
-            const double bo = (double)f * (double)cn;
-            d.boosted[sp][row] = bo;
-            key = select_key(bo);
-            d.key[sp][row] = key;
-        }
-        const uint32_t bin = wmode ? win_bin(key, wbase) : (uint32_t)(key >> sel_shift(0));
-        if (owner && (!wmode || bin != 0u)) {
-            atomicAdd(&h[bin], 1u);
-            if (wmode) atomicAdd(&hc[bin >> 6], 1u);
-        }
-    };
+    auto finish_row = [&](bool owner, int row, int cn, float duty, uint32_t cbw) { overlap_finish_row(d, sp, wmode, fold, wbase, h, hc, owner, row, cn, duty, cbw); };
     for (int row0 = first_row0; row0 < d.c1; row0 += nwaves * rpw * U) {
         const bool first = row0 == first_row0;
         int cnt[U];
@@ -135,22 +167,90 @@
     OV_STAMP(3);
     lds_barrier();
     OV_STAMP(4);
-    uint32_t *g0 = d.hist0 + (size_t)sp * HIST0_PAR + (size_t)(blk & (HIST_REP - 1)) * SEL_BINS;
-    uint32_t *gc = d.hist0 + (size_t)sp * HIST0_PAR + HIST0_FINE + (size_t)(blk & (COARSE_REP - 1)) * COARSE_STRIDE;
-    const int n_fine = wmode ? SEL_BINS - SEL_COARSE : SEL_BINS;
-    {
-        constexpr int PER = SEL_BINS / BS;
-        uint32_t v[PER];
-#pragma unroll
-        for (int k = 0; k < PER; ++k) v[k] = h[threadIdx.x + k * BS];
-#pragma unroll
-        for (int k = 0; k < PER; ++k) {
-            const int i = threadIdx.x + k * BS;
-            if (v[k] && i < n_fine) atomicAdd(&g0[i], v[k]);
-        }
-    }
-    if (wmode && threadIdx.x < SEL_COARSE && hc[threadIdx.x]) atomicAdd(&gc[threadIdx.x], hc[threadIdx.x]);
+    overlap_flush<BS>(d, sp, wmode, blk, h, hc);
     OV_STAMP(5);
+}
+
+#define PLANE_MAX_BYTES 256
+#define PLANE_BATCH 16
+template <int BS>
+__device__ __forceinline__ bool role_overlap_planes(const Dev &d, const uint32_t *__restrict__ bank, int n_inputs, int p, int sp, int step_offset,
+                                                    int blk, int nblk, uint32_t *h, int wmode, int fold, int dense_above) {
+    static_assert(BS >= PLANE_MAX_BYTES && BS % 64 == 0, "one thread per input byte lists the row in one pass");
+    __shared__ uint16_t s_list[PLANE_MAX_BYTES];
+    __shared__ uint32_t s_nz[BS / 64];
+    const int NB = 4 * d.W;
+    if (NB > PLANE_MAX_BYTES) return false;
+    const int gtid = blk * BS + threadIdx.x;
+    const int nthreads = nblk * BS;
+    const uint32_t *in = bank;
+    if (n_inputs > 1) in = bank + (size_t)((d.ctr->step[p] + (uint32_t)step_offset) % (uint32_t)n_inputs) * d.W;
+    const uint32_t byte = (int)threadIdx.x < NB ? (uint32_t)((const uint8_t *)in)[threadIdx.x] : 0u;
+    const int ngroups = d.Cp >> 2;
+    float dty[4] = {0.f, 0.f, 0.f, 0.f};
+    uint32_t cbw = 0u;
+    if (gtid < ngroups) {
+#pragma unroll
+        for (int u = 0; u < 4; ++u) dty[u] = 4 * gtid + u < d.C ? d.duty[4 * gtid + u] : 0.f;
+        if (fold) cbw = d.colbits[p][gtid >> 3];
+    }
+    for (int i = threadIdx.x; i < SEL_BINS; i += BS) h[i] = 0;
+    const u64 nzm = __ballot(byte != 0u);
+    if (lane_id() == 0) s_nz[threadIdx.x >> 6] = (uint32_t)__popcll(nzm);
+    lds_barrier();
+    int n = 0, pos = (int)__popcll(nzm & lanemask_lt());
+#pragma unroll
+    for (int i = 0; i < BS / 64; ++i) {
+        const int t = (int)s_nz[i];
+        if (i < (int)(threadIdx.x >> 6)) pos += t;
+        n += t;
+    }
+    if (n > dense_above) return false;
+    if (byte != 0u) s_list[pos] = (uint16_t)(threadIdx.x | (byte << 8));
+    uint32_t *ghist = d.hist + sp * SEL_MAX_PASSES * SEL_BINS;
+    if (gtid == 0) {
+        d.ctr->emit_epoch += 1;
+        d.ctr->sel_pass_prefix[sp][0] = 0;
+        d.ctr->sel_pass_krem[sp][0] = (uint32_t)d.sel_k;
+    }
+    for (int i = gtid; i < (d.sel_passes - 1) * SEL_BINS; i += nthreads) ghist[SEL_BINS + i] = 0;
+    const uint32_t wbase = wmode ? d.ctr->sel_win[sp] : 0u;
+    lds_barrier();
+    uint32_t *hc = h + SEL_BINS - SEL_COARSE;
+    const uint32_t *planes = (const uint32_t *)d.mask_planes;
+    for (int g = gtid; g < ngroups; g += nthreads) {
+        if (g != gtid) {
+#pragma unroll
+            for (int u = 0; u < 4; ++u) dty[u] = 4 * g + u < d.C ? d.duty[4 * g + u] : 0.f;
+            if (fold) cbw = d.colbits[p][g >> 3];
+        }
+        int cnt[4] = {0, 0, 0, 0};
+        for (int i0 = 0; i0 < n; i0 += PLANE_BATCH) {
+            uint32_t v[PLANE_BATCH];
+#pragma unroll
+            for (int u = 0; u < PLANE_BATCH; ++u) {
+                const uint32_t j = (uint32_t)s_list[min(i0 + u, n - 1)] & 255u;
+                v[u] = planes[(size_t)j * (size_t)ngroups + (size_t)g];
+            }
+#pragma unroll
+            for (int u = 0; u < PLANE_BATCH; ++u) {
+                const uint32_t b = i0 + u < n ? (uint32_t)s_list[min(i0 + u, n - 1)] >> 8 : 0u;
+                const uint32_t x = v[u] & (b * 0x01010101u);
+                cnt[0] += __popc(x & 0x000000FFu);
+                cnt[1] += __popc(x & 0x0000FF00u);
+                cnt[2] += __popc(x & 0x00FF0000u);
+                cnt[3] += __popc(x & 0xFF000000u);
+            }
+        }
+#pragma unroll
+        for (int u = 0; u < 4; ++u) {
+            const int row = 4 * g + u;
+            overlap_finish_row(d, sp, wmode, fold, wbase, h, hc, row >= d.c0 && row < d.c1, row, cnt[u], dty[u], cbw);
+        }
+    }
+    lds_barrier();
+    overlap_flush<BS>(d, sp, wmode, blk, h, hc);
+    return true;
 }
 
 __global__ __launch_bounds__(RB) void k_sp_overlap(Dev d, const uint32_t *__restrict__ bank, int n_inputs, int G, int p, int sp, int step_offset, int wmode) {
@@ -1168,6 +1268,8 @@
     for (int i0 = 0; i0 < d.Ipad; i0 += 256) {
         int i = i0 + threadIdx.x;
         bool conn = false;
+        const bool stores = lane_id() == 0 && i < d.Ipad;
+        const u64 old = stores ? *(const u64 *)&mrow[i >> 5] : 0ull;
         if (i < d.I) {
             bool on = (in[i >> 5] >> (i & 31)) & 1u;
             double v = prow[i] + (on ? d.sp_don : d.sp_doff);
@@ -1175,7 +1277,10 @@
             conn = v >= d.sp_thr;
         }
         u64 m = __ballot(conn);
-        if (lane_id() == 0 && i < d.Ipad) *(u64 *)&mrow[i >> 5] = m;
+        if (stores) {
+            *(u64 *)&mrow[i >> 5] = m;
+            planes_store_changed(d, row, i >> 3, old, m);
+        }
     }
 }
 
diff --git a/bithtm_amd/csrc/htm_tm_kernels.h b/bithtm_amd/csrc/htm_tm_kernels.h
--- a/bithtm_amd/csrc/htm_tm_kernels.h
+++ b/bithtm_amd/csrc/htm_tm_kernels.h
@@ -129,6 +129,10 @@
     for (int i0 = 0; i0 < d.Ipad; i0 += 2 * TPR) {
         const int e0 = i0 + 2 * t;
         bool c0 = false, c1 = false;
+        const int base = i0 + 2 * (t & ~63);
+        const bool stores = lane_id() == 0 && base < d.Ipad;
+        u64 old0 = 0ull, old1 = 0ull;
+        if (stores) { old0 = *(const u64 *)&mrow[base >> 5]; old1 = *(const u64 *)&mrow[(base >> 5) + 2]; }
         if (e0 < d.Ipad) {
             double2 v = *(double2 *)(prow + e0);
             const uint32_t bits = in[e0 >> 5] >> (e0 & 31);
@@ -146,13 +150,14 @@
             }
         }
         const u64 b0 = __ballot(c0), b1 = __ballot(c1);
-        const int base = i0 + 2 * (t & ~63);
-        if (lane_id() == 0 && base < d.Ipad) {
+        if (stores) {
             u64 *mw = (u64 *)&mrow[base >> 5];
             const u64 m0 = spread32((uint32_t)b0) | (spread32((uint32_t)b1) << 1);
             const u64 m1 = spread32((uint32_t)(b0 >> 32)) | (spread32((uint32_t)(b1 >> 32)) << 1);
             mw[0] = m0;
             mw[1] = m1;
+            planes_store_changed(d, row, base >> 3, old0, m0);
+            planes_store_changed(d, row, (base >> 3) + 8, old1, m1);
         }
         if (i0 == 0) ROW_STAMP(3); else ROW_STAMP(5);
     }
diff --git a/include/bithtm_hip.h b/include/bithtm_hip.h
--- a/include/bithtm_hip.h
+++ b/include/bithtm_hip.h
@@ -97,7 +97,9 @@
     HTM_F_MATCH_INFO = 17,
     HTM_F_MATCH_JITTER = 18,
     HTM_F_CELL_MAX_JITTER = 19,
-    HTM_F_SEG_GID = 20
+    HTM_F_SEG_GID = 20,
+    HTM_F_SP_MASK = 21,
+    HTM_F_SP_MASK_PLANES = 22
 } htm_field;
 
 int htm_create(const htm_config *config, htm_handle **out);
```

After: 40800 timesteps/s. 0.969x the previous value.
